# eladb3/SViT

Measured on AMD Instinct MI355X. Metric: clips/sec (fwd+bwd) SViT 16x224^2 bf16, higher is better.
Workload: dtype bf16; 1 GPU; SViT 16x224^2, 8 clips/GPU, 4 object tokens/frame, fwd+CE+bwd+clip+AdamW; global_batch=8, parallelism=dp1, ranks_seen=1, forced_dp=False, launch=hip-graph replay, input=fp32 clips, resident in the replayed step's input buffers, hip_library=svit_amd/lib/libsvit_hip.so

## Files before the change

include/svit_hip.h:

```cpp
#ifndef SVIT_HIP_H
#define SVIT_HIP_H
#include <stdint.h>
#ifdef __cplusplus
extern "C" {
#endif

#define SVIT_HEAD_DIM 96

int svit_version(void);
const char* svit_arch(void);

enum {
  SVIT_EPI_BF16 = 0,
  SVIT_EPI_GELU = 1,
  SVIT_EPI_RESID = 2,
  SVIT_EPI_F32 = 3,
  SVIT_EPI_DGELU = 4,
  SVIT_EPI_RELQ = 5
};
typedef struct {
  const void* A; int32_t lda;
  const void* W; int32_t ldw;
  const float* bias;
  void* out; int32_t ldo;
  void* out2; int32_t ldo2;
  const void* aux; int32_t ldaux;
  const float* row_scale; int32_t rows_per_sample;
  int32_t M, N, K;
  int32_t epilogue; int32_t accumulate;
  int32_t remap_L, remap_N, remap_off;
  const int32_t* relq_map;
  void* relq_out; int32_t relq_ld;
  int32_t relq_extra, relq_rows;
  float relq_scale;
} svit_gemm_args;
int svit_gemm_nt(const svit_gemm_args* args, void* stream);
int svit_gemm_tn(const void* A, int lda, const void* B, int ldb, float* dW, int lddw,
                 int M, int N, int K, int splits, float* dbias ,
                 void* stream);
#define SVIT_TN_GROUP_MAX 16
typedef struct {
  const void* A; const void* B; float* dW; float* dbias;
  int32_t lda, ldb, lddw, M, N, K;
} svit_tn_problem;
int svit_gemm_tn_grouped(const svit_tn_problem* probs, int count, void* stream);
int svit_gemm_tn_grouped_ex(const svit_tn_problem* probs, int count, int ordered, void* stream);
int svit_gemm_tn_grouped_slab(const svit_tn_problem* probs, int count, float* workspace,
                              int64_t workspace_floats, void* stream);
int64_t svit_gemm_tn_grouped_workspace(const svit_tn_problem* probs, int count);
int svit_colsum_bf16(const void* A, int lda, float* out, int M, int N, void* stream);

int svit_cast_f32_bf16(const float* src, void* dst, int64_t n, void* stream);
int svit_table_interp(const float* M, int rows, int J, const float* tables, float* out32, void* out16, void* stream);
typedef struct svit_table_interp_job {
  const float* M;
  const float* tables;
  float* out32;
  void* out16;
  int32_t rows, J;
} svit_table_interp_job;
int svit_table_interp_batched(const svit_table_interp_job* jobs_dev, int n_jobs, int max_rows, void* stream);
int svit_transpose_cast_batched(const float* src_base, void* dst_base, const int64_t* table,
                                int n_mats, int max_tiles, void* stream);
int svit_transpose_bf16_batched(const void* src_base, void* dst_base, const int64_t* table,
                                int n_mats, int max_tiles, void* stream);
int svit_pad_cast_rows(const float* src, void* dst, int R, int C, int ldd, void* stream);
int svit_scale_cast(const float* src, void* dst, const float* row_scale, int rows_per_sample,
                    int64_t rows, int cols, int gather_L, int gather_N, int gather_off,
                    void* stream);

int svit_reduce_defer(int on, void* stream);
int svit_reduce_flush(void* stream);
int svit_reduce_reset(void* stream);

int svit_layernorm_fwd(const float* x, const float* gamma, const float* beta, void* y_bf16,
                       float* y_f32, float* mean, float* rstd, int64_t rows, int C, float eps,
                       void* stream);
int svit_layernorm_bwd(const void* dy , int dy_is_bf16,
                       const float* x, const float* gamma, const float* mean,
                       const float* rstd, const float* dres, float* dx, void* dx_bf16,
                       const float* row_scale, int rows_per_sample, float* dgamma,
                       float* dbeta, int64_t rows, int C, float* workspace,
                       int64_t workspace_floats, void* stream);

int svit_im2col_patch(const float* video, void* cols, int B, int T, int H, int W, void* stream);
int svit_im2col_patch_u8(const uint8_t* frames, int64_t frames_bytes, const void* lut,
                         const int32_t* crops, void* cols, int B, int T, int Hs, int Ws, int S,
                         void* stream);
int svit_mixup_clips(float* x, const void* mix, int B, int planes, int H, int W, void* stream);
int svit_im2col_patch_u8_mix(const uint8_t* frames, int64_t frames_bytes, const float* lut_f32,
                             const int32_t* crops, const void* mix, void* cols, int B, int T, int Hs,
                             int Ws, int S, void* stream);
int svit_fill_special_tokens(float* x, const float* cls, const float* objq, const float* pos_t,
                             int B, int N, int L, int Tx, int O, int C, int add_pos, void* stream);
int svit_special_token_grads(const float* dx, float* g_cls, float* g_obj, float* g_pos, int B, int N,
                             int L, int Tx, int O, int C, int add_pos, void* stream);

typedef struct {
  const void* qkv; int32_t which;
  const float* conv_w;
  const float* gamma; const float* beta;
  void* out; int32_t ld_out;
  void* pre; float* mean; float* rstd;
  int32_t B, heads, T, H, W, n_obj;
  int32_t stride_hw;
  int32_t mode;
  float eps;
  float out_scale;
  const void* relq_R; const int32_t* relq_map; int32_t relq_lpad; float relq_scale;
} svit_pool_args;
int svit_pool_ln_fwd(const svit_pool_args* a, void* stream);

typedef struct {
  const void* d_main; int32_t main_is_f32; int32_t ld_main;
  const void* d_res; const void* d_extra;
  const void* pre; const float* mean; const float* rstd; const float* gamma;
  void* dpre; float* dgamma; float* dbeta;
  int32_t B, heads, Nout;
  float* workspace; int64_t workspace_floats;
  int32_t main_parts; int64_t main_part_stride;
  int32_t extra_is_bf16;
} svit_pool_ln_bwd_args;
int svit_pool_ln_bwd(const svit_pool_ln_bwd_args* a, void* stream);
typedef struct {
  const void* dpre; const float* conv_w; void* dqkv; int32_t which;
  int32_t B, heads, T, H, W, n_obj, stride_hw;
} svit_pool_dgrad_args;
typedef struct {
  const void* dpre; const void* qkv; int32_t which; float* dw;
  int32_t B, heads, T, H, W, n_obj, stride_hw;
  float* workspace; int64_t workspace_floats;
} svit_pool_wgrad_args;
int svit_pool_ln_fwd_qkv(const svit_pool_args* args3, void* stream);
int svit_pool_weight_sel(const float* src_base, const int64_t* src_off, uint32_t* dst, int n_tables,
                         void* stream);
int svit_pool_ln_fwd_qkv_sel(const svit_pool_args* args3, const uint32_t* const* sel3, void* stream);
int svit_pool_ln_bwd_qkv(const svit_pool_ln_bwd_args* args3, void* stream);
#ifdef SVIT_DIAG_POOL_STREAMING
int svit_pool_conv_dgrad(const svit_pool_dgrad_args* a, void* stream);
int svit_pool_conv_wgrad(const svit_pool_wgrad_args* a, void* stream);
int svit_pool_conv_dgrad_qkv(const svit_pool_dgrad_args* args3, void* stream);
int svit_pool_conv_wgrad_qkv(const svit_pool_wgrad_args* args3, void* stream);
#endif
int svit_pool_conv_bwd_qkv(const svit_pool_dgrad_args* dgrad3, const svit_pool_wgrad_args* wgrad3,
                           void* stream);
int64_t svit_pool_conv_bwd_workspace(const svit_pool_dgrad_args* dgrad3);

typedef struct {
  void* qa; int32_t ld;
  const float* rel_h; const float* rel_w; const float* rel_t;
  const int32_t* idx_h; const int32_t* idx_w; const int32_t* idx_t;
  int32_t B, heads, qt, qh, qw, kt, kh, kw, n_obj;
  float inv_scale;
} svit_relq_args;
int svit_relpos_q_fwd(const svit_relq_args* a, void* stream);
typedef struct {
  const void* qa; const void* dqa; int32_t ld;
  const float* rel_h; const float* rel_w; const float* rel_t;
  const int32_t* idx_h; const int32_t* idx_w; const int32_t* idx_t;
  float* dq_extra;
  float* drel_h; float* drel_w; float* drel_t;
  int32_t rows_h, rows_w, rows_t;
  int32_t B, heads, qt, qh, qw, kt, kh, kw, n_obj;
  float inv_scale;
  float* workspace; int64_t workspace_floats;
} svit_relq_bwd_args;
int svit_relpos_q_bwd(const svit_relq_bwd_args* a, void* stream);
typedef struct {
  const void* P; int32_t ldp; void* qa; int32_t ld;
  const int32_t* idx_h; const int32_t* idx_w; const int32_t* idx_t;
  int32_t row_h, row_w, row_t;
  int32_t B, heads, qt, qh, qw, kt, kh, kw, n_obj;
  float inv_scale;
} svit_relq_gather_args;
int svit_relpos_gather(const svit_relq_gather_args* a, void* stream);
typedef struct {
  const void* dqa; int32_t ld; void* D; int32_t ldd;
  const int32_t* idx_h; const int32_t* idx_w; const int32_t* idx_t;
  int32_t off_h, off_w, off_t;
  int32_t B, heads, qt, qh, qw, kt, kh, kw, n_obj;
  float inv_scale;
} svit_relq_scatter_args;
int svit_relpos_scatter(const svit_relq_scatter_args* a, void* stream);

typedef struct {
  const void* qa; const void* ka; const void* v; void* ctx; float* lse2;
  int32_t B, heads, Nq, Nk, DA; float scale; int32_t bias_cols;
} svit_attn_fwd_args;
int svit_attn_fwd(const svit_attn_fwd_args* a, void* stream);
typedef struct {
  const void* qa; const void* ka; const void* v; const void* ctx; const void* dctx;
  const float* lse2; float* delta;
  void* dqa;
  float* dk; float* dv;
  int32_t B, heads, Nq, Nk, DA, q_splits; float scale;
  int32_t bias_cols;
  void* relD; int32_t relD_ld; const int32_t* relD_map; float relD_scale;
  const void* relR; float* relX;
} svit_attn_bwd_args;
int svit_attn_bwd(const svit_attn_bwd_args* a, void* stream);
int svit_attn_bwd_parts(const svit_attn_bwd_args* a);

int svit_maxpool_fwd(const float* x, float* y, uint8_t* idx, int B, int T, int H, int W,
                     int n_obj, int C, void* stream);
int svit_maxpool_bwd(const float* dy, const uint8_t* idx, float* dx, int B, int T, int H, int W,
                     int n_obj, int C, void* stream);
int svit_maxpool_bwd_bf16(const float* dy, const uint8_t* idx, void* dx_bf16, int B, int T, int H, int W,
                          int n_obj, int C, void* stream);

int svit_sumsq(const float* g, int64_t n, float* sumsq, float* workspace,
               int64_t workspace_floats, void* stream);
int svit_adamw_step(float* p, const float* g, float* m, float* v, int64_t n, const float* sumsq,
                    float max_norm, float lr, float beta1, float beta2, float eps, float wd,
                    int step, float grad_scale, void* stream);

typedef struct {
  float lr[2], weight_decay[2];
  float max_norm, clip_value, grad_scale, reserved;
} svit_step_host;
typedef struct {
  int64_t applied, skipped;
  int32_t consecutive, apply;
  float coef, bc1, bc2_sqrt, sumsq, grad_norm, reserved;
} svit_step_dev;

int svit_adamw_bias_table(float beta1, float beta2, float* table, int64_t capacity, int64_t* n_entries);

int svit_step_guard(const float* g, int64_t n, const svit_step_host* host_rec, svit_step_dev* dev_rec,
                    const float* bias_table, int64_t table_entries, float* workspace, int64_t workspace_floats,
                    void* stream);
int svit_adamw_step_guarded(float* p, const float* g, float* m, float* v, int64_t n, int64_t n_decay,
                            const svit_step_host* host_rec, const svit_step_dev* dev_rec, float beta1, float beta2,
                            float eps, void* stream);

typedef struct {
  const float* tokens; int32_t B, N, C, T, O;
  const float* keep;
  const float* w_proj; const float* b_proj; int32_t n_cls;
  const float* w_box; const float* b_box;
  const float* w_bce; const float* b_bce;
  const float* w_con; const float* b_con;
  float* logits; float* boxes; float* contact; float* xobj;
} svit_head_args;
int svit_head_fwd(const svit_head_args* a, void* stream);
typedef struct {
  svit_head_args f;
  const float* dlogits; const float* dboxes; const float* dcontact; const float* dxobj;
  float* dtokens;
  float* gw_proj; float* gb_proj; float* gw_box; float* gb_box; float* gw_bce; float* gb_bce; float* gw_con; float* gb_con;
  int32_t ordered;
} svit_head_bwd_args;
int svit_head_bwd(const svit_head_bwd_args* g, void* stream);

int svit_haog_loss(const float* pred, const float* tar, const float* contact,
                   const int64_t* contact_tar, float* losses, float* g_l1, float* g_bce,
                   float* g_giou, float* g_contact, int R, int Rc, void* stream);
int svit_haog_loss_bwd(const float* upstream, const float* g_l1, const float* g_bce,
                       const float* g_giou, const float* g_contact, float* dpred,
                       float* dcontact, int R, int Rc, void* stream);

int svit_ce_loss(const float* logits, const int64_t* labels, int B, int C, float* loss, float* dlogits, void* stream);
int svit_ce_loss_soft(const float* logits, const float* target, const int64_t* labels, const void* mix, float on,
                      float off, int B, int C, float* loss, float* dlogits, void* stream);
int svit_step_draws(uint64_t* state, const float* keep, int n_blocks, int per_block, float* scales,
                    int n_drop, float p_drop, float* drop, void* stream);

int svit_ensemble_update(const float* preds, const int64_t* labels, const int64_t* clip_ids,
                         int N, int C, int num_clips, int num_videos, int mode, int repeat,
                         float* video_preds, int64_t* video_labels, int64_t* clip_count,
                         int* err, void* stream);
int svit_topk_correct(const float* video_preds, const int64_t* video_labels, int V, int C,
                      const int* ks, int nk, int* counts, int* err, void* stream);
int svit_debug_set(int key, int val);
int svit_debug_set_tn(int step_us_x100, int atomic_tbs_x100);
int svit_debug_set_tn_tile(int mode);
int svit_debug_set_pool(int key, int val);
int svit_debug_pool_bwd_path(void);
int svit_attn_debug_set(int key, int val);
int svit_debug_reset(void);
#ifdef __cplusplus
}
#endif
#endif
```

svit_amd/csrc/gemm_epilogue.h:

```cpp
#pragma once
#include "common.h"
#ifndef SVIT_EPI_AHEAD
#define SVIT_EPI_AHEAD 1
#endif
#include "../../include/svit_hip.h"

template <bool WAVE_PRIVATE>
__device__ __forceinline__ void nt_epi_sync() {
  if constexpr (WAVE_PRIVATE) asm volatile("s_waitcnt lgkmcnt(0)" ::: "memory");
  else __syncthreads();
}

template <int RB, int NB, int EPI, bool WAVE_PRIVATE = false>
__device__ __forceinline__ void nt_epilogue_wide(const svit_gemm_args& p, f32x16_t (&acc)[RB][NB],
                                                 unsigned char* smem, int m0, int n0, int wm, int wn,
                                                 int lane, int wave) {
  constexpr int WN = 32 * NB, EP_LD = WN + 4, GPR = 4 * NB;
  float* stg = (float*)smem + wave * (16 * EP_LD);
  uint4 aux_ring[3][NB];
  auto fetch_aux = [&](int ih, uint4 (&dst)[NB]) {
    const int i = ih >> 1, half = ih & 1;
#pragma unroll
    for (int it = 0; it < NB; ++it) {
      const int idx = lane + 64 * it, rl = idx / GPR, c8 = idx % GPR;
      const int row = m0 + wm * 32 * RB + i * 32 + half * 16 + rl, col = n0 + wn * WN + c8 * 8;
      dst[it] = make_uint4(0, 0, 0, 0);
      if (row < p.M && col < p.N) dst[it] = *(const uint4*)((const bf16_t*)p.aux + (size_t)row * p.ldaux + col);
    }
  };
  float4 bias_r[NB][2];
#pragma unroll
  for (int it = 0; it < NB; ++it) {
    const int col = n0 + wn * WN + ((lane + 64 * it) % GPR) * 8;
    bias_r[it][0] = bias_r[it][1] = make_float4(0.f, 0.f, 0.f, 0.f);
    if (p.bias && col < p.N) {
      bias_r[it][0] = *(const float4*)(p.bias + col);
      bias_r[it][1] = *(const float4*)(p.bias + col + 4);
    }
  }
  constexpr int AHEAD = SVIT_EPI_AHEAD;
  if (EPI == SVIT_EPI_DGELU) {
    fetch_aux(0, aux_ring[0]);
    if (AHEAD > 1 && 2 * RB > 1) fetch_aux(1, aux_ring[1]);
  }
#pragma unroll
  for (int ih = 0; ih < 2 * RB; ++ih) {
    const int i = ih >> 1, half = ih & 1;
#pragma unroll
    for (int j = 0; j < NB; ++j)
#pragma unroll
      for (int rr = 0; rr < 8; ++rr)
        stg[((rr & 3) + 8 * (rr >> 2) + 4 * (lane >> 5)) * EP_LD + j * 32 + (lane & 31)] =
            acc[i][j][half * 8 + rr];
    if (EPI == SVIT_EPI_DGELU && ih + AHEAD < 2 * RB) fetch_aux(ih + AHEAD, aux_ring[(ih + AHEAD) % 3]);
    nt_epi_sync<WAVE_PRIVATE>();
#pragma unroll
    for (int it = 0; it < NB; ++it) {
      const int idx = lane + 64 * it, rl = idx / GPR, c8 = idx % GPR;
      const int row = m0 + wm * 32 * RB + i * 32 + half * 16 + rl, col = n0 + wn * WN + c8 * 8;
      if (row >= p.M || col >= p.N) continue;
      const float4 v0 = *(const float4*)(stg + rl * EP_LD + c8 * 8), v1 = *(const float4*)(stg + rl * EP_LD + c8 * 8 + 4);
      const float4 b0 = bias_r[it][0], b1 = bias_r[it][1];
      float v[8] = {v0.x + b0.x, v0.y + b0.y, v0.z + b0.z, v0.w + b0.w, v1.x + b1.x, v1.y + b1.y, v1.z + b1.z, v1.w + b1.w};
      uint4 o;
      if constexpr (EPI == SVIT_EPI_BF16) {
        o.x = pack_bf16x2(v[0], v[1]); o.y = pack_bf16x2(v[2], v[3]);
        o.z = pack_bf16x2(v[4], v[5]); o.w = pack_bf16x2(v[6], v[7]);
      } else if constexpr (EPI == SVIT_EPI_GELU) {
        float a[8], d[8];
#pragma unroll
        for (int e = 0; e < 8; ++e) gelu_fwd_grad(v[e], &a[e], &d[e]);
        if (p.out2) {
          uint4 o2;
          o2.x = pack_bf16x2(d[0], d[1]); o2.y = pack_bf16x2(d[2], d[3]);
          o2.z = pack_bf16x2(d[4], d[5]); o2.w = pack_bf16x2(d[6], d[7]);
          *(uint4*)((bf16_t*)p.out2 + (size_t)row * p.ldo2 + col) = o2;
        }
        o.x = pack_bf16x2(a[0], a[1]); o.y = pack_bf16x2(a[2], a[3]);
        o.z = pack_bf16x2(a[4], a[5]); o.w = pack_bf16x2(a[6], a[7]);
      } else {
        const uint4 h = aux_ring[ih % 3][it];
        o.x = pack_bf16x2(v[0] * lo_bf16(h.x), v[1] * hi_bf16(h.x));
        o.y = pack_bf16x2(v[2] * lo_bf16(h.y), v[3] * hi_bf16(h.y));
        o.z = pack_bf16x2(v[4] * lo_bf16(h.z), v[5] * hi_bf16(h.z));
        o.w = pack_bf16x2(v[6] * lo_bf16(h.w), v[7] * hi_bf16(h.w));
      }
      *(uint4*)((bf16_t*)p.out + (size_t)row * p.ldo + col) = o;
    }
    if (ih + 1 < 2 * RB) nt_epi_sync<WAVE_PRIVATE>();
  }
}

template <int RB, int NB>
__device__ __forceinline__ void nt_epilogue_relq(const svit_gemm_args& p, f32x16_t (&acc)[RB][NB],
                                                 unsigned char* smem, int m0, int n0, int wm, int wn,
                                                 int lane, int wave) {
  constexpr int WN = 32 * NB, EP_LD = WN + 4;
  constexpr int MAXV = 16;
  float* stg = (float*)smem + wave * (16 * EP_LD);
  const int extra = p.relq_extra, sh = extra == 64 ? 6 : 5;
  const int nv = 16 * extra / 64;
  const int c_lo = n0 + wn * WN;
  bf16_t* qa = (bf16_t*)p.relq_out;
  int cols[2 * RB][MAXV];
#pragma unroll
  for (int ih = 0; ih < 2 * RB; ++ih) {
    const int row0 = m0 + wm * 32 * RB + (ih >> 1) * 32 + (ih & 1) * 16;
    const int tok0 = row0 % p.relq_rows;
#pragma unroll
    for (int it = 0; it < MAXV; ++it) {
      const int e = it * 64 + lane, rl = e >> sh, j = e & (extra - 1);
      cols[ih][it] = -2;
      if (it < nv && row0 + rl < p.M) {
        int tok = tok0 + rl;
        while (tok >= p.relq_rows) tok -= p.relq_rows;
        cols[ih][it] = p.relq_map[tok * extra + j];
      }
    }
  }
#pragma unroll
  for (int ih = 0; ih < 2 * RB; ++ih) {
    const int i = ih >> 1, half = ih & 1;
#pragma unroll
    for (int j = 0; j < NB; ++j)
#pragma unroll
      for (int rr = 0; rr < 8; ++rr)
        stg[((rr & 3) + 8 * (rr >> 2) + 4 * (lane >> 5)) * EP_LD + j * 32 + (lane & 31)] =
            acc[i][j][half * 8 + rr];
    nt_epi_sync<true>();
    const int row0 = m0 + wm * 32 * RB + i * 32 + half * 16;
#pragma unroll
    for (int it = 0; it < MAXV; ++it) {
      const int e = it * 64 + lane, rl = e >> sh, j = e & (extra - 1), col = cols[ih][it];
      if (col == -2) continue;
      const size_t o = (size_t)(row0 + rl) * p.relq_ld + 96 + j;
      if (col < 0) {
        if (c_lo == 0) qa[o] = 0;
      } else if (col >= c_lo && col < c_lo + WN) {
        qa[o] = f32_to_bf16(bf16_to_f32(f32_to_bf16(stg[rl * EP_LD + col - c_lo])) * p.relq_scale);
      }
    }
    if (ih + 1 < 2 * RB) nt_epi_sync<true>();
  }
}

template <int RB, int NB, int EPI, bool WAVE_PRIVATE = false>
__device__ __forceinline__ void nt_epilogue(const svit_gemm_args& p, f32x16_t (&acc)[RB][NB],
                                            unsigned char* smem, int m0, int n0, int wm, int wn,
                                            int lane, int wave) {
  if constexpr (EPI == SVIT_EPI_RELQ) {
    nt_epilogue_relq<RB, NB>(p, acc, smem, m0, n0, wm, wn, lane, wave);
    return;
  }
  if constexpr (EPI == SVIT_EPI_BF16 || EPI == SVIT_EPI_GELU || EPI == SVIT_EPI_DGELU) {
    const bool rows16 = (p.ldo % 8 == 0) && (EPI != SVIT_EPI_GELU || !p.out2 || p.ldo2 % 8 == 0) &&
                        (EPI != SVIT_EPI_DGELU || p.ldaux % 8 == 0);
    if (rows16) {
      nt_epilogue_wide<RB, NB, EPI, WAVE_PRIVATE>(p, acc, smem, m0, n0, wm, wn, lane, wave);
      return;
    }
  }
  constexpr int WN = 32 * NB;
  constexpr int EP_LD = WN + 4;
  constexpr int NIT = 2 * NB;
  constexpr bool HAS_AUX = (EPI == SVIT_EPI_RESID || EPI == SVIT_EPI_DGELU || EPI == SVIT_EPI_F32);
  float* stg = (float*)smem + wave * (16 * EP_LD);
  float4 aux_ring[3][NIT];
  constexpr int AHEAD = SVIT_EPI_AHEAD;
  const bool use_aux = HAS_AUX && (EPI != SVIT_EPI_F32 || p.accumulate);
  auto out_row = [&](int row) -> size_t {
    if (EPI == SVIT_EPI_F32 && p.remap_L > 0)
      return (size_t)(row / p.remap_L) * p.remap_N + p.remap_off + (row % p.remap_L);
    return (size_t)row;
  };
  auto fetch_aux = [&](int ih, float4 (&dst)[NIT]) {
    const int i = ih >> 1, half = ih & 1;
#pragma unroll
    for (int it = 0; it < NIT; ++it) {
      const int idx = lane + 64 * it;
      const int rl = idx / (8 * NB), c4 = idx % (8 * NB);
      const int row = m0 + wm * 32 * RB + i * 32 + half * 16 + rl;
      const int col = n0 + wn * WN + c4 * 4;
      dst[it] = make_float4(0.f, 0.f, 0.f, 0.f);
      if (row >= p.M || col >= p.N) continue;
      if constexpr (EPI == SVIT_EPI_RESID) {
        dst[it] = *(const float4*)((const float*)p.aux + (size_t)row * p.ldaux + col);
      } else if constexpr (EPI == SVIT_EPI_DGELU) {
        const uint2 h = *(const uint2*)((const bf16_t*)p.aux + (size_t)row * p.ldaux + col);
        dst[it].x = __uint_as_float(h.x);
        dst[it].y = __uint_as_float(h.y);
      } else if constexpr (EPI == SVIT_EPI_F32) {
        dst[it] = *(const float4*)((const float*)p.out + out_row(row) * p.ldo + col);
      }
    }
  };
  float4 bias_r[NIT];
#pragma unroll
  for (int it = 0; it < NIT; ++it) {
    const int col = n0 + wn * WN + ((lane + 64 * it) % (8 * NB)) * 4;
    bias_r[it] = make_float4(0.f, 0.f, 0.f, 0.f);
    if (p.bias && col < p.N) bias_r[it] = *(const float4*)(p.bias + col);
  }
  float rs_lo = 1.f, rs_hi = 1.f;
  int rs_boundary = 0x7fffffff;
  const bool rs_fast = EPI == SVIT_EPI_RESID && p.row_scale && p.rows_per_sample >= 32 * RB;
  if (rs_fast) {
    const int r_first = min(m0 + wm * 32 * RB, p.M - 1), r_last = min(r_first + 32 * RB - 1, p.M - 1);
    rs_lo = p.row_scale[r_first / p.rows_per_sample];
    rs_hi = p.row_scale[r_last / p.rows_per_sample];
    rs_boundary = (r_first / p.rows_per_sample + 1) * p.rows_per_sample;
  }
  if (use_aux) {
    fetch_aux(0, aux_ring[0]);
    if (AHEAD > 1 && 2 * RB > 1) fetch_aux(1, aux_ring[1]);
  }
#pragma unroll
  for (int ih = 0; ih < 2 * RB; ++ih) {
    const int i = ih >> 1, half = ih & 1;
#pragma unroll
    for (int j = 0; j < NB; ++j)
#pragma unroll
      for (int rr = 0; rr < 8; ++rr)
        stg[((rr & 3) + 8 * (rr >> 2) + 4 * (lane >> 5)) * EP_LD + j * 32 + (lane & 31)] =
            acc[i][j][half * 8 + rr];
    if (use_aux && ih + AHEAD < 2 * RB) fetch_aux(ih + AHEAD, aux_ring[(ih + AHEAD) % 3]);
    nt_epi_sync<WAVE_PRIVATE>();
#pragma unroll
    for (int it = 0; it < NIT; ++it) {
      const int idx = lane + 64 * it;
      const int rl = idx / (8 * NB), c4 = idx % (8 * NB);
      const int row = m0 + wm * 32 * RB + i * 32 + half * 16 + rl;
      const int col = n0 + wn * WN + c4 * 4;
      if (row >= p.M || col >= p.N) continue;
      float4 v = *(const float4*)(stg + rl * EP_LD + c4 * 4);
      {
        const float4 b = bias_r[it];
        v.x += b.x; v.y += b.y; v.z += b.z; v.w += b.w;
      }
      if constexpr (EPI == SVIT_EPI_BF16) {
        uint2 o;
        o.x = pack_bf16x2(v.x, v.y); o.y = pack_bf16x2(v.z, v.w);
        *(uint2*)((bf16_t*)p.out + (size_t)row * p.ldo + col) = o;
      } else if constexpr (EPI == SVIT_EPI_GELU) {
        float a0, a1, a2, a3, d0, d1, d2, d3;
        gelu_fwd_grad(v.x, &a0, &d0); gelu_fwd_grad(v.y, &a1, &d1);
        gelu_fwd_grad(v.z, &a2, &d2); gelu_fwd_grad(v.w, &a3, &d3);
        uint2 o;
        if (p.out2) {
          o.x = pack_bf16x2(d0, d1); o.y = pack_bf16x2(d2, d3);
          *(uint2*)((bf16_t*)p.out2 + (size_t)row * p.ldo2 + col) = o;
        }
        o.x = pack_bf16x2(a0, a1); o.y = pack_bf16x2(a2, a3);
        *(uint2*)((bf16_t*)p.out + (size_t)row * p.ldo + col) = o;
      } else if constexpr (EPI == SVIT_EPI_RESID) {
        const float s = rs_fast ? (row < rs_boundary ? rs_lo : rs_hi)
                                : (p.row_scale ? p.row_scale[row / p.rows_per_sample] : 1.f);
        const float4 res = aux_ring[ih % 3][it];
        float4 o;
        o.x = res.x + s * v.x; o.y = res.y + s * v.y; o.z = res.z + s * v.z; o.w = res.w + s * v.w;
        *(float4*)((float*)p.out + (size_t)row * p.ldo + col) = o;
      } else if constexpr (EPI == SVIT_EPI_F32) {
        float4* o = (float4*)((float*)p.out + out_row(row) * p.ldo + col);
        if (p.accumulate) {
          const float4 old = aux_ring[ih % 3][it];
          v.x += old.x; v.y += old.y; v.z += old.z; v.w += old.w;
        }
        *o = v;
      } else if constexpr (EPI == SVIT_EPI_DGELU) {
        const uint32_t hx = __float_as_uint(aux_ring[ih % 3][it].x), hy = __float_as_uint(aux_ring[ih % 3][it].y);
        uint2 o;
        o.x = pack_bf16x2(v.x * lo_bf16(hx), v.y * hi_bf16(hx));
        o.y = pack_bf16x2(v.z * lo_bf16(hy), v.w * hi_bf16(hy));
        *(uint2*)((bf16_t*)p.out + (size_t)row * p.ldo + col) = o;
      }
    }
    if (ih + 1 < 2 * RB) nt_epi_sync<WAVE_PRIVATE>();
  }
}
```

svit_amd/csrc/gemm_nt.hip:

```cpp
#include "gemm_epilogue.h"
#include "attn_common.h"

namespace {

template <int BK>
__device__ __forceinline__ int nt_lds_off(int r, int ch) {
  if constexpr (BK == 32) return r * 64 + 16 * (ch ^ ((r >> 2) & 3));
  else return (r >> 4) * 2048 + (r & 7) * 256 + ((r >> 3) & 1) * 128 + 16 * (ch ^ (r & 7));
}

template <int N>
__device__ __forceinline__ void wait_vmcnt() {
  asm volatile("s_waitcnt vmcnt(%0)" ::"n"(N) : "memory");
}

template <int RB, int NB, int WAVES_M, int WAVES_N, int STAGES, int EPI, int BK2>
__global__ __launch_bounds__(WAVES_M* WAVES_N * 64, (WAVES_M * WAVES_N > 4 ? 1 : 2)) void
gemm_nt_v2_kernel(svit_gemm_args p) {
  constexpr int NT = WAVES_M * WAVES_N * 64;
  constexpr int BM = 32 * RB * WAVES_M, WN = 32 * NB, BN = WN * WAVES_N;
  constexpr int CPR = BK2 / 8;
  constexpr int RPR = NT / CPR;
  constexpr int ROWS = (BM + BN + RPR - 1) / RPR * RPR;
  constexpr int STAGE_BYTES = ROWS * BK2 * 2;
  constexpr int PER = ROWS * CPR / NT;
  extern __shared__ __attribute__((aligned(16))) unsigned char smem[];

  const int tid = threadIdx.x, lane = tid & 63, wave = tid >> 6;
  const int wm = wave / WAVES_N, wn = wave % WAVES_N;
  const int nwg = gridDim.x * gridDim.y, lin = blockIdx.y * gridDim.x + blockIdx.x;
  const int xq = nwg >> 3, xr = nwg & 7, xcd = lin & 7;
  const int wgid = (xcd < xr ? xcd * (xq + 1) : xr * (xq + 1) + (xcd - xr) * xq) + (lin >> 3);
  const int m0 = (wgid / gridDim.x) * BM, n0 = (wgid % gridDim.x) * BN;

  const bf16_t* src[PER];
#pragma unroll
  for (int i = 0; i < PER; ++i) {
    const int q = tid + i * NT;
    int row, ch;
    if constexpr (BK2 == 32) {
      row = q >> 2;
      ch = (q & 3) ^ ((row >> 2) & 3);
    } else {
      const int line = q >> 4;
      row = (line >> 3) * 16 + ((q >> 3) & 1) * 8 + (line & 7);
      ch = (q & 7) ^ (row & 7);
    }
    if (row < BM) {
      const int gr = min(m0 + row, p.M - 1);
      src[i] = (const bf16_t*)p.A + (size_t)gr * p.lda + ch * 8;
    } else {
      const int gr = min(n0 + row - BM, p.N - 1);
      src[i] = (const bf16_t*)p.W + (size_t)gr * p.ldw + ch * 8;
    }
  }
  auto issue = [&](int kt, int stage) {
    unsigned char* base = smem + stage * STAGE_BYTES + wave * 1024;
#pragma unroll
    for (int i = 0; i < PER; ++i)
      __builtin_amdgcn_global_load_lds(
          (const __attribute__((address_space(1))) void*)(src[i] + kt * BK2),
          (__attribute__((address_space(3))) void*)(base + i * (NT * 16)), 16, 0, 0);
  };

  f32x16_t acc[RB][NB];
#pragma unroll
  for (int i = 0; i < RB; ++i)
#pragma unroll
    for (int j = 0; j < NB; ++j)
#pragma unroll
      for (int r = 0; r < 16; ++r) acc[i][j][r] = 0.f;

  const int nk = p.K / BK2;
#pragma unroll
  for (int s = 0; s < STAGES - 1; ++s)
    if (s < nk) issue(s, s);

  const int a_row = wm * 32 * RB + (lane & 31);
  const int w_row = BM + wn * WN + (lane & 31);
  for (int kt = 0; kt < nk; ++kt) {
    if (kt + STAGES - 2 < nk) wait_vmcnt<(STAGES - 2) * PER>();
    else wait_vmcnt<0>();
    __builtin_amdgcn_s_barrier();
    if (kt + STAGES - 1 < nk) issue(kt + STAGES - 1, (kt + STAGES - 1) % STAGES);
    const unsigned char* st = smem + (kt % STAGES) * STAGE_BYTES;
    bf16x8_t af[BK2 / 16][RB], wf[BK2 / 16][NB];
#pragma unroll
    for (int ks = 0; ks < BK2 / 16; ++ks) {
      const int ch = 2 * ks + (lane >> 5);
#pragma unroll
      for (int i = 0; i < RB; ++i) {
        const int r = a_row + i * 32;
        af[ks][i] = *(const bf16x8_t*)(st + nt_lds_off<BK2>(r, ch));
      }
#pragma unroll
      for (int j = 0; j < NB; ++j) {
        const int r = w_row + j * 32;
        wf[ks][j] = *(const bf16x8_t*)(st + nt_lds_off<BK2>(r, ch));
      }
    }
    __builtin_amdgcn_sched_barrier(0);
#pragma unroll
    for (int ks = 0; ks < BK2 / 16; ++ks)
#pragma unroll
      for (int i = 0; i < RB; ++i)
#pragma unroll
        for (int j = 0; j < NB; ++j) acc[i][j] = mfma32(af[ks][i], wf[ks][j], acc[i][j]);
    __builtin_amdgcn_sched_barrier(0);
  }
  __syncthreads();
  nt_epilogue<RB, NB, EPI, true>(p, acc, smem, m0, n0, wm, wn, lane, wave);
}

template <int RB, int NB, int WAVES_M, int WAVES_N, int STAGES, int BK2 = 32>
int launch_v2(const svit_gemm_args& a, hipStream_t st) {
  constexpr int BM = 32 * RB * WAVES_M, BN = 32 * NB * WAVES_N;
  constexpr int NT = WAVES_M * WAVES_N * 64;
  constexpr int RPR = NT / (BK2 / 8);
  size_t lds = (size_t)STAGES * ((BM + BN + RPR - 1) / RPR * RPR) * BK2 * 2;
  const size_t lds_epi = (size_t)WAVES_M * WAVES_N * 16 * (32 * NB + 4) * sizeof(float);
  if (lds < lds_epi) lds = lds_epi;
  dim3 grid((a.N + BN - 1) / BN, (a.M + BM - 1) / BM);
  static SvitOnce once[6];
#define SVIT_V2_ATTR(E)                                                                              \
  if (int rc = svit_max_lds_once(once[E], (const void*)gemm_nt_v2_kernel<RB, NB, WAVES_M, WAVES_N, STAGES, E, BK2>, lds)) \
    return rc
  SVIT_V2_ATTR(SVIT_EPI_BF16); SVIT_V2_ATTR(SVIT_EPI_GELU); SVIT_V2_ATTR(SVIT_EPI_RESID);
  SVIT_V2_ATTR(SVIT_EPI_F32); SVIT_V2_ATTR(SVIT_EPI_DGELU); SVIT_V2_ATTR(SVIT_EPI_RELQ);
#undef SVIT_V2_ATTR
#define SVIT_V2_CASE(E)                                                                       \
  case E:                                                                                     \
    hipLaunchKernelGGL((gemm_nt_v2_kernel<RB, NB, WAVES_M, WAVES_N, STAGES, E, BK2>), grid, dim3(NT), \
                       lds, st, a);                                                           \
    break;
  switch (a.epilogue) {
    SVIT_V2_CASE(SVIT_EPI_BF16)
    SVIT_V2_CASE(SVIT_EPI_GELU)
    SVIT_V2_CASE(SVIT_EPI_RESID)
    SVIT_V2_CASE(SVIT_EPI_F32)
    SVIT_V2_CASE(SVIT_EPI_DGELU)
    SVIT_V2_CASE(SVIT_EPI_RELQ)
    default:
      return SVIT_ERR_ARG;
  }
#undef SVIT_V2_CASE
  SVIT_LAUNCH_CHECK();
  return SVIT_OK;
}

template <int NL, int BM, int BN, int STAGES>
__device__ __forceinline__ void nt_ring_loader(const svit_gemm_args& p, unsigned char* smem, int lw, int lane,
                                               int m0, int n0, int nk) {
  constexpr int PIECES = (BM + BN) / 8;
  constexpr int PER = (PIECES + NL - 1) / NL;
  constexpr int STAGE_BYTES = (BM + BN) * 128;
  const bf16_t* src[PER];
  auto piece_of = [&](int i) { return min(lw + NL * i, PIECES - 1); };
#pragma unroll
  for (int i = 0; i < PER; ++i) {
    const int q = piece_of(i) * 64 + lane, line = q >> 4;
    const int row = (line >> 3) * 16 + ((q >> 3) & 1) * 8 + (line & 7);
    const int ch = (q & 7) ^ (row & 7);
    if (row < BM) src[i] = (const bf16_t*)p.A + (size_t)min(m0 + row, p.M - 1) * p.lda + ch * 8;
    else src[i] = (const bf16_t*)p.W + (size_t)min(n0 + row - BM, p.N - 1) * p.ldw + ch * 8;
  }
  auto issue = [&](int kt) {
    unsigned char* st = smem + (kt % STAGES) * STAGE_BYTES;
#pragma unroll
    for (int i = 0; i < PER; ++i)
      __builtin_amdgcn_global_load_lds((const __attribute__((address_space(1))) void*)(src[i] + kt * 64),
                                       (__attribute__((address_space(3))) void*)(st + piece_of(i) * 1024), 16, 0, 0);
  };
#pragma unroll
  for (int s = 0; s < STAGES; ++s)
    if (s < nk) issue(s);
  for (int kt = 0; kt < nk; ++kt) {
    const int younger = (kt == 0 ? min(STAGES - 1, nk - 1) : min(kt + STAGES - 2, nk - 1) - kt);
    attn::static_for<0, STAGES>([&](auto Y) {
      if (younger == decltype(Y)::value) wait_vmcnt<decltype(Y)::value * PER>();
    });
    __builtin_amdgcn_s_barrier();
    if (kt >= 1 && kt - 1 + STAGES < nk) issue(kt - 1 + STAGES);
  }
}

template <int RB, int NB, int WAVES_M, int WAVES_N, int NL, int STAGES, int EPI>
__global__ __launch_bounds__((WAVES_M * WAVES_N + NL) * 64, 1) void gemm_nt_ring_kernel(svit_gemm_args p) {
  using attn::Int;
  constexpr int NC = WAVES_M * WAVES_N;
  constexpr int BM = 32 * RB * WAVES_M, WN = 32 * NB, BN = WN * WAVES_N;
  static_assert(BM % 16 == 0 && BN % 16 == 0, "a 1-KiB piece must not straddle A and W rows");
  constexpr int STAGE_BYTES = (BM + BN) * 128;
  extern __shared__ __attribute__((aligned(16))) unsigned char smem[];

  const int lane = threadIdx.x & 63;
  const int wave = __builtin_amdgcn_readfirstlane(threadIdx.x >> 6);
  const int nwg = gridDim.x * gridDim.y, lin = blockIdx.y * gridDim.x + blockIdx.x;
  const int xq = nwg >> 3, xr = nwg & 7, xcd = lin & 7;
  const int wgid = (xcd < xr ? xcd * (xq + 1) : xr * (xq + 1) + (xcd - xr) * xq) + (lin >> 3);
  const int m0 = (wgid / gridDim.x) * BM, n0 = (wgid % gridDim.x) * BN;
  const int nk = p.K / 64;

  if (wave >= NC) {
    nt_ring_loader<NL, BM, BN, STAGES>(p, smem, wave - NC, lane, m0, n0, nk);
    return;
  }

  const int wm = wave / WAVES_N, wn = wave % WAVES_N;
  f32x16_t acc[RB][NB];
#pragma unroll
  for (int i = 0; i < RB; ++i)
#pragma unroll
    for (int j = 0; j < NB; ++j)
#pragma unroll
      for (int r = 0; r < 16; ++r) acc[i][j][r] = 0.f;

  const int l31 = lane & 31, x7 = lane & 7;
  unsigned fa[4], fw[4];
#pragma unroll
  for (int ks = 0; ks < 4; ++ks) {
    const unsigned lp = (unsigned)((l31 >> 4) * 2048 + x7 * 256 + ((l31 >> 3) & 1) * 128 +
                                   32 * (ks ^ (x7 >> 1)) + 16 * ((lane >> 5) ^ (x7 & 1)));
    fa[ks] = (unsigned)(size_t)smem + lp + (unsigned)(wm * 2 * RB) * 2048u;
    fw[ks] = (unsigned)(size_t)smem + lp + (unsigned)((BM + wn * WN) / 16) * 2048u;
  }
  bf16x8_t fr[2][RB + NB];
  auto reads = [&](auto KS, auto BUF, unsigned so, auto HALF) {
    constexpr int ks = decltype(KS)::value, b = decltype(BUF)::value, h = decltype(HALF)::value;
    attn::static_for<0, RB + NB>([&](auto F) {
      constexpr int f = decltype(F)::value;
      if constexpr ((f / 2) == h) {
        if constexpr (f < RB) attn::lds_read128<f * 4096>(fr[b][f], fa[ks] + so);
        else attn::lds_read128<(f - RB) * 4096>(fr[b][f], fw[ks] + so);
      }
    });
  };
  constexpr int NH = (RB + NB + 1) / 2;
  auto release = [&](auto BUF) {
    constexpr int b = decltype(BUF)::value;
    attn::static_for<0, RB + NB>([&](auto F) { attn::lgkm_release1<0>(fr[b][decltype(F)::value]); });
  };
  auto substep = [&](auto BUF, auto NEXT_KS, unsigned next_so, bool do_reads) {
    constexpr int b = decltype(BUF)::value;
    attn::static_for<0, RB * NB>([&](auto Q) {
      constexpr int q = decltype(Q)::value, i = q / NB, j = q % NB;
      acc[i][j] = mfma32(fr[b][i], fr[b][RB + j], acc[i][j]);
      if constexpr (q < NH) {
        if (do_reads) reads(NEXT_KS, Int<1 - b>{}, next_so, Int<q>{});
      }
      __builtin_amdgcn_sched_barrier(0);
    });
  };

  __builtin_amdgcn_s_barrier();
  attn::static_for<0, NH>([&](auto H) { reads(Int<0>{}, Int<0>{}, 0u, H); });
  release(Int<0>{});
  for (int kt = 0; kt < nk; ++kt) {
    const unsigned so = (unsigned)((kt % STAGES) * STAGE_BYTES);
    const unsigned so_next = (unsigned)(((kt + 1) % STAGES) * STAGE_BYTES);
    const bool more = kt + 1 < nk;
    substep(Int<0>{}, Int<1>{}, so, true);
    release(Int<1>{});
    substep(Int<1>{}, Int<2>{}, so, true);
    release(Int<0>{});
    substep(Int<0>{}, Int<3>{}, so, true);
    release(Int<1>{});
    if (more) __builtin_amdgcn_s_barrier();
    substep(Int<1>{}, Int<0>{}, so_next, more);
    if (more) release(Int<0>{});
  }
  unsigned char* epi = smem + (nk >= 2 ? (nk - 2) % STAGES : 1) * STAGE_BYTES;
  nt_epilogue<RB, NB, EPI, true>(p, acc, epi, m0, n0, wm, wn, lane, wave);
}

template <int RB, int NB, int WAVES_M, int WAVES_N, int NL, int STAGES>
int launch_ring(const svit_gemm_args& a, hipStream_t st) {
  constexpr int BM = 32 * RB * WAVES_M, BN = 32 * NB * WAVES_N, NT = (WAVES_M * WAVES_N + NL) * 64;
  constexpr size_t lds = (size_t)STAGES * (BM + BN) * 128;
  static_assert((size_t)WAVES_M * WAVES_N * 16 * (32 * NB + 4) * sizeof(float) <= (size_t)(BM + BN) * 128, "epilogue staging fits a slot");
  static_assert(lds <= 160 * 1024, "LDS");
  dim3 grid((a.N + BN - 1) / BN, (a.M + BM - 1) / BM);
  static SvitOnce once[5];
#define SVIT_RING_ATTR(E)                                                                              \
  if (int rc = svit_max_lds_once(once[E], (const void*)gemm_nt_ring_kernel<RB, NB, WAVES_M, WAVES_N, NL, STAGES, E>, lds)) \
    return rc
  SVIT_RING_ATTR(SVIT_EPI_BF16); SVIT_RING_ATTR(SVIT_EPI_GELU); SVIT_RING_ATTR(SVIT_EPI_RESID);
  SVIT_RING_ATTR(SVIT_EPI_F32); SVIT_RING_ATTR(SVIT_EPI_DGELU);
#undef SVIT_RING_ATTR
#define SVIT_RING_CASE(E)                                                                       \
  case E:                                                                                       \
    hipLaunchKernelGGL((gemm_nt_ring_kernel<RB, NB, WAVES_M, WAVES_N, NL, STAGES, E>), grid, dim3(NT), lds, st, a); \
    break;
  switch (a.epilogue) {
    SVIT_RING_CASE(SVIT_EPI_BF16)
    SVIT_RING_CASE(SVIT_EPI_GELU)
    SVIT_RING_CASE(SVIT_EPI_RESID)
    SVIT_RING_CASE(SVIT_EPI_F32)
    SVIT_RING_CASE(SVIT_EPI_DGELU)
    default:
      return SVIT_ERR_ARG;
  }
#undef SVIT_RING_CASE
  SVIT_LAUNCH_CHECK();
  return SVIT_OK;
}
}

static void ring_choice(const svit_gemm_args& a, int* cfg, int* stages) {
  const long tm = (a.M + 127) / 128;
  const long t192 = a.N % 192 == 0 ? tm * (a.N / 192) : 0, t96 = tm * ((a.N + 95) / 96);
  constexpr int k_min5 = 1024, t_max6 = 256, s6 = 4;
  if (t96 <= t_max6 && a.K >= 768) { *cfg = 6, *stages = (t96 > 256 ? 2 : s6); return; }
  if (t192 >= 160 && a.N <= 768 && a.K >= k_min5) { *cfg = 5, *stages = 3; return; }
}

extern "C" int svit_gemm_nt(const svit_gemm_args* args, void* stream) {
  if (!args || !args->A || !args->W) return SVIT_ERR_ARG;
  const svit_gemm_args& a = *args;
  const bool relq = a.epilogue == SVIT_EPI_RELQ;
  if (!relq && !a.out) return SVIT_ERR_ARG;
  if (relq) {
    if (!a.relq_map || !a.relq_out || (a.relq_extra != 32 && a.relq_extra != 64) || a.relq_rows < 1 ||
        a.relq_ld < 96 + a.relq_extra || a.bias)
      return SVIT_ERR_ARG;
  }
  if (a.M <= 0 || a.N <= 0 || a.K <= 0 || a.K % 32 != 0 || a.N % 96 != 0) return SVIT_ERR_SHAPE;
  if (a.lda % 8 != 0 || a.ldw % 8 != 0 || a.lda < a.K || a.ldw < a.K || (!relq && a.ldo < a.N))
    return SVIT_ERR_ALIGN;
  if (((uintptr_t)a.A | (uintptr_t)a.W) & 15) return SVIT_ERR_ALIGN;
  if (!relq && (a.ldo % 4 != 0 || ((uintptr_t)a.out & 15))) return SVIT_ERR_ALIGN;
  if (a.bias && ((uintptr_t)a.bias & 15)) return SVIT_ERR_ALIGN;
  if (a.aux && (a.ldaux % 4 != 0 || ((uintptr_t)a.aux & 15))) return SVIT_ERR_ALIGN;
  if (a.out2 && (a.ldo2 % 4 != 0 || ((uintptr_t)a.out2 & 15))) return SVIT_ERR_ALIGN;
  if ((a.epilogue == SVIT_EPI_RESID || a.epilogue == SVIT_EPI_DGELU) && !a.aux) return SVIT_ERR_ARG;
  if (a.epilogue == SVIT_EPI_RESID && a.row_scale && a.rows_per_sample <= 0) return SVIT_ERR_ARG;
  hipStream_t st = (hipStream_t)stream;
  const int force_raw = svit_knob(SVIT_K_NT_CFG), force_stages = svit_knob(SVIT_K_NT_STAGES);
  const bool no_ring = force_raw == 8 || svit_knob(SVIT_K_NT_BK) != 0;
  const int force_cfg = force_raw == 8 ? -1 : force_raw;
  if (a.K % 64 == 0 && !relq && ((force_cfg < 0 && !no_ring) || (force_cfg >= 5 && force_cfg <= 7))) {
    int cfg = force_cfg, rs = force_stages;
    if (cfg < 0) ring_choice(a, &cfg, &rs);
    if (cfg >= 5) {
      if (!rs) rs = 3;
#define SVIT_RING_PICK(RB, NB, WM, WN)                                         \
  do {                                                                         \
    if (rs == 2) return launch_ring<RB, NB, WM, WN, 4, 2>(a, st);              \
    if (rs == 3) return launch_ring<RB, NB, WM, WN, 4, 3>(a, st);              \
    return launch_ring<RB, NB, WM, WN, 4, 4>(a, st);                           \
  } while (0)
      if (cfg == 5) SVIT_RING_PICK(2, 3, 2, 2);
      if (cfg == 6) SVIT_RING_PICK(1, 3, 4, 1);
      SVIT_RING_PICK(2, 2, 2, 2);
#undef SVIT_RING_PICK
    }
  }
  bool big = a.N % 192 == 0 && (long)((a.M + 127) / 128) * (a.N / 192) >= 256;
  if (force_cfg == 0 && a.N % 192 == 0) big = true;
  if (force_cfg == 2) big = false;
  const int stages = force_stages ? force_stages : (a.K >= 2048 ? 4 : 2);
  bool sq = a.N % 128 == 0 && a.N >= 1024 && a.K <= 512 &&
            (long)((a.M + 127) / 128) * (a.N / 128) <= 2048;
  if (force_cfg == 4) sq = a.N % 128 == 0;
  else if (force_cfg >= 0) sq = false;
  const int force_bk = svit_knob(SVIT_K_NT_BK);
  bool bk64 = a.K % 64 == 0 && a.N <= 768 && a.K >= 384;
  if (force_bk) bk64 = force_bk == 64 && a.K % 64 == 0;
  if (bk64 && force_cfg < 0 && !force_stages) return launch_v2<1, 3, 4, 1, 2, 64>(a, st);
#define SVIT_NT_PICK(RB, NB, WM, WN)                                           \
  do {                                                                         \
    if (bk64) {                                                                \
      if (stages == 2) return launch_v2<RB, NB, WM, WN, 2, 64>(a, st);         \
      if (stages == 3) return launch_v2<RB, NB, WM, WN, 3, 64>(a, st);         \
      return launch_v2<RB, NB, WM, WN, 4, 64>(a, st);                          \
    }                                                                          \
    if (stages == 2) return launch_v2<RB, NB, WM, WN, 2, 32>(a, st);           \
    if (stages == 3) return launch_v2<RB, NB, WM, WN, 3, 32>(a, st);           \
    return launch_v2<RB, NB, WM, WN, 4, 32>(a, st);                            \
  } while (0)
  {
    constexpr int one_round = 1;
    const long t160 = a.N % 256 == 0 ? (long)((a.M + 159) / 160) * (a.N / 256) : 0;
    const long t192 = a.N % 192 == 0 ? (long)((a.M + 191) / 192) * (a.N / 192) : 0;
    const long t128 = (long)((a.M + 127) / 128) * ((a.N + 191) / 192);
    const bool auto_ok = force_cfg < 0 && one_round && !force_stages && !force_bk && a.K <= 512 && t128 > 512;
    if (force_cfg == 9 || (auto_ok && t160 > 256 && t160 <= 512)) {
      if (a.N % 256 == 0) return launch_v2<5, 2, 1, 4, 2, 32>(a, st);
    }
    if (force_cfg == 10 || (auto_ok && t192 > 256 && t192 <= 512)) {
      if (a.N % 192 == 0) return launch_v2<3, 3, 2, 2, 2, 32>(a, st);
    }
  }
  if (sq) SVIT_NT_PICK(2, 2, 2, 2);
  if (big) SVIT_NT_PICK(2, 3, 2, 2);
  SVIT_NT_PICK(1, 3, 4, 1);
#undef SVIT_NT_PICK
}
```

svit_amd/csrc/norm.hip:

```cpp
#include <algorithm>
#include <cstdlib>
#include "common.h"
#include "../../include/svit_hip.h"

namespace {
constexpr int LN_MAX_CHUNKS = 3;

template <bool HALF>
__device__ __forceinline__ float row_sum(float v) {
#pragma unroll
  for (int o = HALF ? 16 : 32; o > 0; o >>= 1) v += __shfl_xor(v, o, 64);
  return v;
}

template <int NCH, bool HALF>
__global__ __launch_bounds__(256) void ln_fwd_kernel(const float* __restrict__ x,
                                                     const float* __restrict__ gamma,
                                                     const float* __restrict__ beta,
                                                     bf16_t* __restrict__ y16,
                                                     float* __restrict__ y32,
                                                     float* __restrict__ mean_out,
                                                     float* __restrict__ rstd_out, int64_t rows,
                                                     int C, float eps) {
  constexpr int LW = HALF ? 32 : 64;
  constexpr int RPW = HALF ? 2 : 1;
  const int lane = threadIdx.x & 63, wave = threadIdx.x >> 6;
  const int lr = lane & (LW - 1), sub = HALF ? (lane >> 5) : 0;
  const int nch = C >> 2;
  const float inv_c = 1.0f / (float)C;
  float4 g[NCH], bt[NCH];
#pragma unroll
  for (int i = 0; i < NCH; ++i) {
    const int c = lr + i * LW;
    g[i] = bt[i] = make_float4(0.f, 0.f, 0.f, 0.f);
    if (c < nch) { g[i] = ((const float4*)gamma)[c]; bt[i] = ((const float4*)beta)[c]; }
  }
  const int64_t stride = (int64_t)gridDim.x * 4 * RPW;
  for (int64_t row0 = ((int64_t)blockIdx.x * 4 + wave) * RPW + sub; row0 < rows; row0 += 2 * stride) {
    float4 v[2][NCH];
    int64_t rk[2];
    bool has[2];
#pragma unroll
    for (int k = 0; k < 2; ++k) {
      has[k] = row0 + k * stride < rows;
      rk[k] = has[k] ? row0 + k * stride : row0;
#pragma unroll
      for (int i = 0; i < NCH; ++i) {
        const int c = lr + i * LW;
        v[k][i] = make_float4(0.f, 0.f, 0.f, 0.f);
        if (c < nch) v[k][i] = ((const float4*)(x + rk[k] * C))[c];
      }
    }
#pragma unroll
    for (int k = 0; k < 2; ++k) {
      float s = 0.f;
#pragma unroll
      for (int i = 0; i < NCH; ++i) s += v[k][i].x + v[k][i].y + v[k][i].z + v[k][i].w;
      const float mean = row_sum<HALF>(s) * inv_c;
      float sq = 0.f;
#pragma unroll
      for (int i = 0; i < NCH; ++i) {
        if (lr + i * LW < nch) {
          const float a = v[k][i].x - mean, b = v[k][i].y - mean, cc = v[k][i].z - mean,
                      d = v[k][i].w - mean;
          sq += a * a + b * b + cc * cc + d * d;
        }
      }
      const float rstd = rsqrtf(row_sum<HALF>(sq) * inv_c + eps);
      if (!has[k]) continue;
      if (lr == 0) {
        if (mean_out) mean_out[rk[k]] = mean;
        if (rstd_out) rstd_out[rk[k]] = rstd;
      }
#pragma unroll
      for (int i = 0; i < NCH; ++i) {
        const int c = lr + i * LW;
        if (c < nch) {
          float4 o;
          o.x = (v[k][i].x - mean) * rstd * g[i].x + bt[i].x;
          o.y = (v[k][i].y - mean) * rstd * g[i].y + bt[i].y;
          o.z = (v[k][i].z - mean) * rstd * g[i].z + bt[i].z;
          o.w = (v[k][i].w - mean) * rstd * g[i].w + bt[i].w;
          if (y16) {
            uint2 pk;
            pk.x = pack_bf16x2(o.x, o.y);
            pk.y = pack_bf16x2(o.z, o.w);
            *(uint2*)(y16 + rk[k] * C + c * 4) = pk;
          }
          if (y32) ((float4*)(y32 + rk[k] * C))[c] = o;
        }
      }
    }
  }
}

template <int NCH, bool HALF, bool DYB>
__global__ __launch_bounds__(256) void ln_bwd_kernel(const void* __restrict__ dy_,
                                                     const float* __restrict__ x,
                                                     const float* __restrict__ gamma,
                                                     const float* __restrict__ mean_in,
                                                     const float* __restrict__ rstd_in,
                                                     const float* __restrict__ dres,
                                                     float* __restrict__ dx,
                                                     bf16_t* __restrict__ dx16,
                                                     const float* __restrict__ row_scale,
                                                     int rows_per_sample,
                                                     float* __restrict__ partial,
                                                     int64_t rows, int C) {
  constexpr int LW = HALF ? 32 : 64;
  constexpr int RPW = HALF ? 2 : 1;
  __shared__ float red[4][2][NCH * 256];
  const int lane = threadIdx.x & 63, wave = threadIdx.x >> 6;
  const int lr = lane & (LW - 1), sub = HALF ? (lane >> 5) : 0;
  const int nch = C >> 2;
  const float inv_c = 1.0f / (float)C;
  float4 gacc[NCH], bacc[NCH], gm[NCH];
#pragma unroll
  for (int i = 0; i < NCH; ++i) {
    gacc[i] = make_float4(0.f, 0.f, 0.f, 0.f);
    bacc[i] = make_float4(0.f, 0.f, 0.f, 0.f);
    const int c = lr + i * LW;
    gm[i] = (c < nch) ? ((const float4*)gamma)[c] : make_float4(0.f, 0.f, 0.f, 0.f);
  }
  const int64_t stride = (int64_t)gridDim.x * 4 * RPW;
  for (int64_t row0 = ((int64_t)blockIdx.x * 4 + wave) * RPW + sub; row0 < rows; row0 += 2 * stride) {
    float4 xv[2][NCH], dv[2][NCH], rv[2][NCH];
    float mean[2], rstd[2], sc16[2];
    int64_t rowk[2];
    bool has[2];
#pragma unroll
    for (int k = 0; k < 2; ++k) {
      has[k] = row0 + k * stride < rows;
      rowk[k] = has[k] ? row0 + k * stride : row0;
      mean[k] = mean_in[rowk[k]];
      rstd[k] = rstd_in[rowk[k]];
      sc16[k] = (dx16 && row_scale) ? row_scale[rowk[k] / rows_per_sample] : 1.f;
#pragma unroll
      for (int i = 0; i < NCH; ++i) {
        const int c = lr + i * LW;
        xv[k][i] = dv[k][i] = rv[k][i] = make_float4(0.f, 0.f, 0.f, 0.f);
        if (c < nch) {
          xv[k][i] = ((const float4*)(x + rowk[k] * C))[c];
          if (DYB) {
            const uint2 h = ((const uint2*)((const bf16_t*)dy_ + rowk[k] * C))[c];
            dv[k][i] = make_float4(lo_bf16(h.x), hi_bf16(h.x), lo_bf16(h.y), hi_bf16(h.y));
          } else {
            dv[k][i] = ((const float4*)((const float*)dy_ + rowk[k] * C))[c];
          }
          if (dres) rv[k][i] = ((const float4*)(dres + rowk[k] * C))[c];
        }
      }
    }
#pragma unroll
    for (int k = 0; k < 2; ++k) {
      float4 xh[NCH], g[NCH];
      float s1 = 0.f, s2 = 0.f;
      const float live = has[k] ? 1.f : 0.f;
#pragma unroll
      for (int i = 0; i < NCH; ++i) {
        const float4 d = dv[k][i];
        xh[i].x = (xv[k][i].x - mean[k]) * rstd[k]; xh[i].y = (xv[k][i].y - mean[k]) * rstd[k];
        xh[i].z = (xv[k][i].z - mean[k]) * rstd[k]; xh[i].w = (xv[k][i].w - mean[k]) * rstd[k];
        if (lr + i * LW >= nch) xh[i] = make_float4(0.f, 0.f, 0.f, 0.f);
        gacc[i].x += live * d.x * xh[i].x; gacc[i].y += live * d.y * xh[i].y;
        gacc[i].z += live * d.z * xh[i].z; gacc[i].w += live * d.w * xh[i].w;
        bacc[i].x += live * d.x; bacc[i].y += live * d.y;
        bacc[i].z += live * d.z; bacc[i].w += live * d.w;
        g[i].x = d.x * gm[i].x; g[i].y = d.y * gm[i].y;
        g[i].z = d.z * gm[i].z; g[i].w = d.w * gm[i].w;
        s1 += g[i].x + g[i].y + g[i].z + g[i].w;
        s2 += g[i].x * xh[i].x + g[i].y * xh[i].y + g[i].z * xh[i].z + g[i].w * xh[i].w;
      }
      s1 = row_sum<HALF>(s1) * inv_c;
      s2 = row_sum<HALF>(s2) * inv_c;
      if (!has[k]) continue;
#pragma unroll
      for (int i = 0; i < NCH; ++i) {
        const int c = lr + i * LW;
        if (c < nch) {
          float4 o;
          o.x = rstd[k] * (g[i].x - s1 - xh[i].x * s2) + rv[k][i].x;
          o.y = rstd[k] * (g[i].y - s1 - xh[i].y * s2) + rv[k][i].y;
          o.z = rstd[k] * (g[i].z - s1 - xh[i].z * s2) + rv[k][i].z;
          o.w = rstd[k] * (g[i].w - s1 - xh[i].w * s2) + rv[k][i].w;
          ((float4*)(dx + rowk[k] * C))[c] = o;
          if (dx16) {
            uint2 h;
            h.x = pack_bf16x2(o.x * sc16[k], o.y * sc16[k]);
            h.y = pack_bf16x2(o.z * sc16[k], o.w * sc16[k]);
            ((uint2*)(dx16 + rowk[k] * C))[c] = h;
          }
        }
      }
    }
  }
  if (HALF) {
#pragma unroll
    for (int i = 0; i < NCH; ++i) {
      gacc[i].x += __shfl_xor(gacc[i].x, 32, 64); gacc[i].y += __shfl_xor(gacc[i].y, 32, 64);
      gacc[i].z += __shfl_xor(gacc[i].z, 32, 64); gacc[i].w += __shfl_xor(gacc[i].w, 32, 64);
      bacc[i].x += __shfl_xor(bacc[i].x, 32, 64); bacc[i].y += __shfl_xor(bacc[i].y, 32, 64);
      bacc[i].z += __shfl_xor(bacc[i].z, 32, 64); bacc[i].w += __shfl_xor(bacc[i].w, 32, 64);
    }
  }
#pragma unroll
  for (int i = 0; i < NCH; ++i) {
    const int c = lr + i * LW;
    if (c < nch && sub == 0) {
      *(float4*)&red[wave][0][c * 4] = gacc[i];
      *(float4*)&red[wave][1][c * 4] = bacc[i];
    }
  }
  __syncthreads();
  float* prow = partial + (size_t)blockIdx.x * 2 * C;
  for (int c = threadIdx.x; c < C; c += 256) {
    prow[c] = red[0][0][c] + red[1][0][c] + red[2][0][c] + red[3][0][c];
    prow[C + c] = red[0][1][c] + red[1][1][c] + red[2][1][c] + red[3][1][c];
  }
}
}

extern "C" int svit_layernorm_fwd(const float* x, const float* gamma, const float* beta,
                                  void* y_bf16, float* y_f32, float* mean, float* rstd,
                                  int64_t rows, int C, float eps, void* stream) {
  if (!x || !gamma || !beta || (!y_bf16 && !y_f32)) return SVIT_ERR_ARG;
  if (rows <= 0 || C <= 0 || C % 4 != 0 || C > 768) return SVIT_ERR_SHAPE;
  constexpr int rpb_f = 8;
  int64_t blocks = (rows + rpb_f - 1) / rpb_f;
  if (blocks > 16384) blocks = 16384;
  if (blocks < 1) blocks = 1;
#define SVIT_LN_FWD(NCH, HALF)                                                                \
  hipLaunchKernelGGL((ln_fwd_kernel<NCH, HALF>), dim3((unsigned)blocks), dim3(256), 0,           \
                     (hipStream_t)stream, x, gamma, beta, (bf16_t*)y_bf16, y_f32, mean, rstd,    \
                     rows, C, eps)
  if (C <= 128) SVIT_LN_FWD(1, true);
  else if (C <= 256) SVIT_LN_FWD(1, false);
  else if (C <= 512) SVIT_LN_FWD(2, false);
  else SVIT_LN_FWD(3, false);
#undef SVIT_LN_FWD
  SVIT_LAUNCH_CHECK();
  return SVIT_OK;
}

extern "C" int svit_layernorm_bwd(const void* dy, int dy_is_bf16, const float* x, const float* gamma,
                                  const float* mean, const float* rstd, const float* dres,
                                  float* dx, void* dx_bf16, const float* row_scale,
                                  int rows_per_sample, float* dgamma, float* dbeta, int64_t rows,
                                  int C, float* workspace, int64_t workspace_floats,
                                  void* stream) {
  if (!dy || !x || !gamma || !mean || !rstd || !dx || !dgamma || !dbeta || !workspace)
    return SVIT_ERR_ARG;
  if (dx_bf16 && row_scale && rows_per_sample <= 0) return SVIT_ERR_ARG;
  if (rows <= 0 || C <= 0 || C % 4 != 0 || C > 768) return SVIT_ERR_SHAPE;
  constexpr int rpb = 16;
  int64_t blocks = (rows + rpb - 1) / rpb;
  if (blocks < 256) blocks = (rows + 3) / 4 < 256 ? (rows + 3) / 4 : 256;
  if (blocks > 2048) blocks = 2048;
  if (blocks > workspace_floats / (2 * C)) blocks = workspace_floats / (2 * C);
  if (blocks < 1) return SVIT_ERR_ARG;
#define SVIT_LN_BWD(NCH, HALF)                                                                  \
  do {                                                                                            \
    if (dy_is_bf16)                                                                               \
      hipLaunchKernelGGL((ln_bwd_kernel<NCH, HALF, true>), dim3((unsigned)blocks), dim3(256), 0,  \
                         (hipStream_t)stream, dy, x, gamma, mean, rstd, dres, dx,                 \
                         (bf16_t*)dx_bf16, row_scale, rows_per_sample, workspace, rows, C);       \
    else                                                                                          \
      hipLaunchKernelGGL((ln_bwd_kernel<NCH, HALF, false>), dim3((unsigned)blocks), dim3(256), 0, \
                         (hipStream_t)stream, dy, x, gamma, mean, rstd, dres, dx,                 \
                         (bf16_t*)dx_bf16, row_scale, rows_per_sample, workspace, rows, C);       \
  } while (0)
  if (C <= 128) SVIT_LN_BWD(1, true);
  else if (C <= 256) SVIT_LN_BWD(1, false);
  else if (C <= 512) SVIT_LN_BWD(2, false);
  else SVIT_LN_BWD(3, false);
#undef SVIT_LN_BWD
  SVIT_LAUNCH_CHECK();
  SvitReduceDst dst = {{dgamma, dbeta, dbeta, dbeta, dbeta, dbeta}, {C, 2 * C, 2 * C, 2 * C, 2 * C, 2 * C}};
  svit_launch_reduce(workspace, (int)blocks, 2 * C, dst, (hipStream_t)stream);
  SVIT_LAUNCH_CHECK();
  return SVIT_OK;
}
```

svit_amd/engine.py:

```python
import math

import torch

from . import arch, hip, ops
from .input import U8Clips

HD = arch.HEAD_DIM
F32, BF16 = torch.float32, torch.bfloat16
SCALE = HD ** -0.5
LOG2E = 1.4426950408889634
K_SCALE = SCALE * LOG2E


def _align(n, a=8):
    return (n + a - 1) // a * a


class FlatParams:

    def __init__(self, shapes, decay_of, device, rank_of):
        names = list(shapes)
        depth = 1 + max([int(n.split(".")[1]) for n in names if n.startswith("blocks.")] or [0])
        ranks = {n: rank_of(n, depth) for n in names}
        order = sorted(names, key=lambda n: (not decay_of(n, shapes[n]), ranks[n]))
        self.slots, off = {}, 0
        self.n_decay = 0
        self.n_ranks = depth + 2
        self.ready_ranges = [[] for _ in range(self.n_ranks)]
        for n in order:
            numel = int(math.prod(shapes[n]))
            self.slots[n] = (off, numel, tuple(shapes[n]))
            rr = self.ready_ranges[ranks[n]]
            if rr and rr[-1][1] == off:
                rr[-1] = (rr[-1][0], off + _align(numel))
            else:
                rr.append((off, off + _align(numel)))
            off += _align(numel)
            if decay_of(n, shapes[n]):
                self.n_decay = off
        self.total = off
        self.data = torch.zeros(off, device=device, dtype=F32)
        self.grad = torch.zeros(off, device=device, dtype=F32)
        self.w16 = torch.zeros(off + 96 * 96, device=device, dtype=BF16)
        self.t_slots, toff, table = {}, 0, []
        for n in order:
            if n.startswith("blocks.") and n.endswith(".weight") and len(shapes[n]) == 2:
                r, c = shapes[n]
                self.t_slots[n] = (toff, (c, r))
                table += [self.slots[n][0], toff, r, c, r]
                toff += _align(r * c)
        self.rel_slots = {}
        for n in order:
            if n.endswith("attn.rel_pos_h"):
                pre = n[:-len("attn.rel_pos_h")]
                rows = [shapes[pre + "attn.rel_pos_" + a][0] for a in "hwt"]
                offs, lpad = rel_sections(rows)
                self.rel_slots[pre] = (toff, lpad, offs)
                for a, o, r in zip("hwt", offs, rows):
                    table += [self.slots[pre + "attn.rel_pos_" + a][0], toff + o, r, HD, lpad]
                toff += _align(HD * lpad)
        pool_names = [n for n in names if ".attn.pool_" in n and n.endswith(".weight")]
        pool_names.sort(key=lambda n: (int(n.split(".")[1]), "qkv".index(n.split(".")[3][-1])))
        self.pool_sel_index = {n: i for i, n in enumerate(pool_names)}
        self.pool_sel = torch.zeros((max(1, len(pool_names)), 27 * 96), device=device, dtype=torch.int32)
        self.pool_sel_off = torch.tensor([self.slots[n][0] for n in pool_names] or [0], dtype=torch.int64,
                                         device=device)
        self.wT16 = torch.zeros(max(toff, 8), device=device, dtype=BF16)
        self.t_table = torch.tensor(table, dtype=torch.int64, device=device)
        self.n_t = len(table) // 5

    def view(self, buf, name):
        off, numel, shape = self.slots[name]
        return buf[off:off + numel].view(shape)

    def p(self, name):
        return self.view(self.data, name)

    def g(self, name):
        return self.view(self.grad, name)

    def w(self, name):
        off, numel, shape = self.slots[name]
        return self.w16[off:off + numel].view(shape)

    def wt(self, name):
        off, shape = self.t_slots[name]
        return self.wT16[off:off + shape[0] * shape[1]].view(shape)

    def rel_cat_t(self, pre):
        off, lpad, offs = self.rel_slots[pre]
        return self.wT16[off:off + HD * lpad].view(HD, lpad), lpad, offs

    def rel_tables32(self, pre):
        names = [pre + "attn.rel_pos_" + a for a in "hwt"]
        offs = [self.slots[n][0] for n in names]
        rows = [self.slots[n][2][0] for n in names]
        assert offs[1] == offs[0] + rows[0] * HD and offs[2] == offs[1] + rows[1] * HD
        return self.data[offs[0]:offs[0] + sum(rows) * HD].view(sum(rows), HD)

    def rel_cat(self, pre):
        names = [pre + "attn.rel_pos_" + a for a in "hwt"]
        offs = [self.slots[n][0] for n in names]
        rows = [self.slots[n][2][0] for n in names]
        assert offs[1] == offs[0] + rows[0] * HD and offs[2] == offs[1] + rows[1] * HD
        total = rows[0] + rows[1] + rows[2]
        lpad = (total + 95) // 96 * 96
        return (self.w16[offs[0]:offs[0] + lpad * HD].view(lpad, HD), (0, rows[0], rows[0] + rows[1]))

    def sels(self, pre):
        return [self.pool_sel[self.pool_sel_index[pre + "attn.pool_%s.weight" % r]] for r in "qkv"]

    TILED_MIN_PLANE = 2048
    SLAB_MAX_PLANE = 196

    def refresh_low_precision(self):
        ops.cast_bf16(self.data, self.w16[:self.total])
        if self.pool_sel_index:
            ops.pool_weight_sel(self.data, self.pool_sel_off, self.pool_sel)
        if self.n_t:
            ops.transpose_bf16_batched(self.w16, self.wT16, self.t_table, self.n_t, 256)


def rel_sections(rows):
    off_w = _align(rows[0])
    off_t = off_w + _align(rows[1])
    return (0, off_w, off_t), _align(off_t + rows[2], 32)


def _rel_index(q_n, k_n):
    q_ratio = max(k_n / q_n, 1.0)
    k_ratio = max(q_n / k_n, 1.0)
    d = torch.arange(q_n)[:, None] * q_ratio - torch.arange(k_n)[None, :] * k_ratio
    d = d + (k_n - 1) * k_ratio
    return d.long().to(torch.int32)


def _resize_matrix(rows_have, rows_need):
    m = torch.zeros(rows_need, rows_have)
    scale = rows_have / rows_need
    for i in range(rows_need):
        pos = max((i + 0.5) * scale - 0.5, 0.0)
        i0 = min(int(math.floor(pos)), rows_have - 1)
        i1 = min(i0 + 1, rows_have - 1)
        lam = pos - i0
        m[i, i0] += 1.0 - lam
        m[i, i1] += lam
    return m


class Engine:
    def __init__(self, plan: arch.Plan, flat: FlatParams, red_group=4):
        self.plan, self.flat = plan, flat
        self.dev = flat.data.device
        self._rel_cache = {}
        self._interp_cache = {}
        self._interp_out = {}
        self.batch_interp = True
        self._relq_cache = {}
        self.fused_scatter = True
        self.patch_w16 = torch.zeros((plan.embed_dim, 448), device=self.dev, dtype=BF16)
        self._tn = []
        self.RED_GROUP = max(1, int(red_group))
        M1 = 1024 * 1024
        self._red_ws = torch.empty(self.RED_GROUP * 18 * M1, device=self.dev, dtype=F32)
        self._red_slot = 0
        self._wgrad_need, self._wgrad_big = {}, {}
        self._red_regions = {"ln2": (0, 4 * M1), "ln1": (4 * M1, 8 * M1), "pln": (8 * M1, 9 * M1),
                             "wgrad": (9 * M1, 18 * M1)}
        self._side = None
        self._side_keep = []
        self._side_active = False
        self.overlap_wgrad = False
        self.attn_q_splits = 0
        self.deterministic = False
        self.reproducible = False
        self._capture_fork = None
        self._capture_join = None

    def refresh_weights(self):
        self.flat.refresh_low_precision()
        ops.pad_cast_rows(self.flat.p("patch_embed.proj.weight").view(self.plan.embed_dim, 441),
                          self.patch_w16)

    def _rel(self, blk, q_thw, k_thw):
        key = (blk.index, q_thw, k_thw)
        ent = self._rel_cache.get(key)
        if ent is None:
            idx = [_rel_index(q_thw[1], k_thw[1]), _rel_index(q_thw[2], k_thw[2]),
                   _rel_index(q_thw[0], k_thw[0])]
            need = [2 * max(q_thw[i], k_thw[i]) - 1 for i in (1, 2, 0)]
            have = [blk.rel_sp_rows, blk.rel_sp_rows, blk.rel_t_rows]
            mats = [None if n == h else _resize_matrix(h, n).to(self.dev) for n, h in zip(need, have)]
            mcat = None
            if any(m is not None for m in mats):
                lp = (sum(need) + 95) // 96 * 96
                mcat = torch.zeros((lp, sum(have)), device=self.dev)
                r0 = c0 = 0
                for n, h, m in zip(need, have, mats):
                    mcat[r0:r0 + n, c0:c0 + h] = torch.eye(h, device=self.dev) if m is None else m
                    r0, c0 = r0 + n, c0 + h
            ent = ([t.contiguous().to(self.dev) for t in idx], mats, mcat, tuple(need))
            self._rel_cache[key] = ent
        return ent

    def _interp_tables(self, thw, save):
        if not self.batch_interp:
            self._interp_out = {}
            return
        key = (tuple(thw), bool(save))
        ent = self._interp_cache.get(key)
        if ent is None:
            entries, outs, cur = [], {}, tuple(thw)
            for blk in self.plan.blocks:
                sq, skv = blk.stride_q[1], blk.stride_kv[1]
                q_thw = (cur[0], arch.pooled(cur[1], sq), arch.pooled(cur[2], sq))
                k_thw = (cur[0], arch.pooled(cur[1], skv), arch.pooled(cur[2], skv))
                _, _, mcat, _ = self._rel(blk, q_thw, k_thw)
                if mcat is not None:
                    r32 = torch.empty((mcat.shape[0], HD), device=self.dev, dtype=F32) if save else None
                    r16 = torch.empty((mcat.shape[0], HD), device=self.dev, dtype=BF16)
                    entries.append((mcat, self.flat.rel_tables32("blocks.%d." % blk.index), r32, r16))
                    outs[blk.index] = (r32, r16)
                cur = q_thw
            jobs = ops.table_interp_jobs(entries, self.dev) if entries else None
            ent = (jobs, max((e[0].shape[0] for e in entries), default=0), outs, entries)
            self._interp_cache[key] = ent
        jobs, max_rows, outs, _ = ent
        if jobs is not None:
            ops.table_interp_batched(jobs, max_rows)
        self._interp_out = outs

    def _relq_map(self, blk, q_thw, k_thw, idx, rows_off, n_obj, extra):
        key = (blk.index, q_thw, k_thw, tuple(rows_off), n_obj, extra)
        m = self._relq_cache.get(key)
        if m is None:
            qt, qh, qw = q_thw
            kt, kh, kw = k_thw
            ih, iw, it = (t.cpu().view(n, k) for t, n, k in zip(idx, (qh, qw, qt), (kh, kw, kt)))
            Lq = qt * qh * qw
            body = torch.full((qt, qh, qw, extra), -1, dtype=torch.int32)
            body[..., :kh] = (rows_off[0] + ih).view(1, qh, 1, kh)
            body[..., kh:kh + kw] = (rows_off[1] + iw).view(1, 1, qw, kw)
            body[..., kh + kw:kh + kw + kt] = (rows_off[2] + it).view(qt, 1, 1, kt)
            m = torch.full((1 + Lq + n_obj, extra), -1, dtype=torch.int32)
            m[1:1 + Lq] = body.view(Lq, extra)
            m = m.contiguous().to(self.dev)
            self._relq_cache[key] = m
        return m

    def _tables(self, pre, mats):
        names = (pre + "attn.rel_pos_h", pre + "attn.rel_pos_w", pre + "attn.rel_pos_t")
        out = []
        for n, m in zip(names, mats):
            t = self.flat.p(n)
            out.append(t if m is None else (m @ t).contiguous())
        return out

    def forward(self, video, drop_scales=None, save=True):
        plan, f = self.plan, self.flat
        if isinstance(video, U8Clips):
            B, _, Tx = video.shape[:3]
            cols, (To, Ho, Wo) = ops.im2col_patch_u8(video)
        else:
            if video.dim() == 4:
                video = video.unsqueeze(2)
            video = video.contiguous().to(F32)
            B, _, Tx = video.shape[:3]
            cols, (To, Ho, Wo) = ops.im2col_patch(video)
        T = plan.num_frames // plan.patch_stride[0] if Tx > 1 else Tx
        if To != T:
            raise hip.SvitHipError("clip has %d frames but cfg.DATA.NUM_FRAMES=%d" % (Tx, plan.num_frames))
        L, n_obj, C = To * Ho * Wo, Tx * plan.objects, plan.embed_dim
        N = 1 + L + n_obj
        x = torch.empty((B, N, C), device=self.dev, dtype=F32)
        ops.gemm_nt(cols, self.patch_w16, f.p("patch_embed.proj.bias"), hip.EPI_F32,
                    out=x.view(B * N, C), remap=(L, N, 1))
        ops.fill_special_tokens(x, f.p("cls_token"), f.p("object_queries"),
                                f.p("pos_embed_temporal"), L, Tx, plan.objects, Tx > 1)
        st = {"B": B, "Tx": Tx, "n_obj": n_obj, "L0": L, "cols": cols if save else None,
              "blocks": []}
        thw = (T, Ho, Wo)
        self._interp_tables(thw, save)
        hip.mark("stem")
        for blk in plan.blocks:
            ds = drop_scales[blk.index] if drop_scales is not None else None
            x, thw, sv = self._block_fwd(blk, x, thw, n_obj, ds, save)
            st["blocks"].append(sv)
            hip.mark("fwd%d" % blk.index)
        y16, y32, mean, rstd = ops.layernorm_fwd(x, f.p("norm.weight"), f.p("norm.bias"),
                                                 want_f32=True, want_bf16=False, save_stats=save)
        st.update(x_last=x if save else None, mean=mean, rstd=rstd, thw=thw)
        self._interp_out = {}
        return y32, st

    def _block_fwd(self, blk, x, thw, n_obj, ds, save):
        f = self.flat
        pre = "blocks.%d." % blk.index
        B, N, C = x.shape
        Co, h = blk.dim_out, blk.heads
        sq, skv = blk.stride_q[1], blk.stride_kv[1]
        q_thw = (thw[0], arch.pooled(thw[1], sq), arch.pooled(thw[2], sq))
        k_thw = (thw[0], arch.pooled(thw[1], skv), arch.pooled(thw[2], skv))
        Nq = 1 + q_thw[0] * q_thw[1] * q_thw[2] + n_obj
        J = k_thw[0] + k_thw[1] + k_thw[2]
        DA = HD + 32 if J <= 32 else HD + 64
        if J > 64:
            raise hip.SvitHipError("key grid %s too large for the in-MFMA rel-pos bias" % (k_thw,))
        xn, _, mean1, rstd1 = ops.layernorm_fwd(x, f.p(pre + "norm1.weight"), f.p(pre + "norm1.bias"),
                                                save_stats=save)
        xn2d = xn.view(B * N, C)
        qkv = ops.gemm_nt(xn2d, f.w(pre + "attn.qkv.weight"), f.p(pre + "attn.qkv.bias"), hip.EPI_BF16)
        idx, mats, mcat, need = self._rel(blk, q_thw, k_thw)
        if mcat is None:
            tabs = self._tables(pre, mats)
            rcat, rows_off = f.rel_cat(pre)
        else:
            if blk.index in self._interp_out:
                r32, rcat = self._interp_out[blk.index]
            else:
                r32, rcat = ops.table_interp(mcat, f.rel_tables32(pre), want_f32=save)
            rows_off = (0, need[0], need[0] + need[1])
            tabs = None if r32 is None else [r32[rows_off[0]:rows_off[0] + need[0]], r32[rows_off[1]:rows_off[1] + need[1]],
                                             r32[rows_off[2]:rows_off[2] + need[2]]]
        pools = ops.pool_ln_fwd_qkv(
            qkv, [f.p(pre + "attn.pool_%s.weight" % r).view(HD, 27) for r in "qkv"],
            [f.p(pre + "attn.norm_%s.weight" % r) for r in "qkv"],
            [f.p(pre + "attn.norm_%s.bias" % r) for r in "qkv"],
            B, h, thw, n_obj, (sq, skv, skv), (DA, DA, HD), (0, 1, 0), save=save, out_scales=(1.0, K_SCALE, 1.0),
            sels=f.sels(pre) if (thw[1] * thw[2] >= f.TILED_MIN_PLANE or thw[1] * thw[2] <= f.SLAB_MAX_PLANE)
            else None,
            relq=(rcat.contiguous(), self._relq_map(blk, q_thw, k_thw, idx, rows_off, n_obj, DA - HD), LOG2E))
        qa, ka, v = pools[0][0], pools[1][0], pools[2][0]
        ctx, lse2 = ops.attn_fwd(qa, ka, v, SCALE, bias_cols=J)
        pool_idx = None
        if blk.has_proj:
            skip = ops.gemm_nt(xn2d, f.w(pre + "proj.weight"), f.p(pre + "proj.bias"), hip.EPI_F32)
            skip = skip.view(B, N, Co)
        else:
            skip = x
        if blk.pools_q:
            skip, pool_idx = ops.maxpool_fwd(skip, thw, n_obj)
        dpa, dpm = ds if ds is not None else (None, None)
        x1 = ops.gemm_nt(ctx.view(B * Nq, Co), f.w(pre + "attn.proj.weight"), f.p(pre + "attn.proj.bias"),
                         hip.EPI_RESID, aux=skip.view(B * Nq, Co), row_scale=dpa, rows_per_sample=Nq)
        x1 = x1.view(B, Nq, Co)
        xn2, _, mean2, rstd2 = ops.layernorm_fwd(x1, f.p(pre + "norm2.weight"), f.p(pre + "norm2.bias"),
                                                 save_stats=save)
        act, dact = ops.gemm_nt(xn2.view(B * Nq, Co), f.w(pre + "mlp.fc1.weight"),
                                f.p(pre + "mlp.fc1.bias"), hip.EPI_GELU, save=save)
        x2 = ops.gemm_nt(act, f.w(pre + "mlp.fc2.weight"), f.p(pre + "mlp.fc2.bias"), hip.EPI_RESID,
                         aux=x1.view(B * Nq, Co), row_scale=dpm, rows_per_sample=Nq).view(B, Nq, Co)
        sv = None
        if save:
            sv = dict(x=x, thw=thw, q_thw=q_thw, k_thw=k_thw, mean1=mean1, rstd1=rstd1, xn=xn2d,
                      qkv=qkv, pools=pools, tabs=tabs, idx=idx, mats=mats, ctx=ctx, lse2=lse2,
                      pool_idx=pool_idx, x1=x1, mean2=mean2, rstd2=rstd2, xn2=xn2, act=act,
                      dact=dact, dpa=dpa, dpm=dpm, Nq=Nq)
        return x2, q_thw, sv

    def backward(self, st, dy, on_ready=None, ready_ranks=None):
        def ready(rank):
            if on_ready is not None:
                if ready_ranks is None or rank in ready_ranks:
                    ops.reduce_flush()
                    self._flush_tn()
                    self._join()
                on_ready(rank)
        plan, f = self.plan, self.flat
        depth = len(plan.blocks)
        last = st["blocks"][depth - 1]
        dx, dx16 = ops.layernorm_bwd(dy.contiguous(), st["x_last"], f.p("norm.weight"), st["mean"],
                                     st["rstd"], f.g("norm.weight"), f.g("norm.bias"),
                                     want_bf16=True, row_scale=last["dpm"],
                                     rows_per_sample=st["x_last"].shape[1])
        ready(0)
        hip.mark("bwd_norm")
        for blk in reversed(plan.blocks):
            below = st["blocks"][blk.index - 1] if blk.index > 0 else None
            try:
                G = self.RED_GROUP
                dx, dx16 = self._block_bwd(blk, st["blocks"][blk.index], dx, dx16, st["n_obj"], below,
                                           red_begin=blk.index % G == G - 1 or blk.index == depth - 1,
                                           red_end=blk.index % G == 0, red_slot=blk.index % G)
            except BaseException:
                ops.reduce_reset()
                self._tn = []
                raise
            hip.mark("bwd%d" % blk.index)
            ready(1 + (depth - 1 - blk.index))
        B, Tx, L, O, C = st["B"], st["Tx"], st["L0"], plan.objects, plan.embed_dim
        ops.special_token_grads(dx, f.g("cls_token"), f.g("object_queries"),
                                f.g("pos_embed_temporal") if Tx > 1 else None, L, Tx, O, Tx > 1)
        dtok = ops.scale_cast(dx, gather=(L, 1))
        self._gemm_tn(dtok, st["cols"], f.g("patch_embed.proj.weight").view(C, 441), f.g("patch_embed.proj.bias"))
        self._flush_tn()
        self._join()
        ready(depth + 1)

    def _rws(self, key):
        a, b = self._red_regions[key]
        o = self._red_slot * 18 * 1024 * 1024
        return self._red_ws[o + a:o + b]

    def _wgrad_ws(self, B, h, thw, n_obj, strides):
        key = (B, h, tuple(thw), n_obj, tuple(strides))
        need = self._wgrad_need.get(key)
        if need is None:
            need = self._wgrad_need[key] = ops.pool_conv_bwd_workspace(B, h, thw, n_obj, strides)
        ws = self._rws("wgrad")
        if need <= ws.numel():
            return ws
        big = self._wgrad_big.get(self._red_slot)
        if big is None or big.numel() < need:
            big = self._wgrad_big[self._red_slot] = torch.empty(need, device=self.dev, dtype=F32)
        return big

    def _fork(self, fn, keep):
        if not self.overlap_wgrad:
            fn()
            return
        if self._capture_fork is not None:
            self._capture_fork(fn)
            self._side_active = True
            return
        main = torch.cuda.current_stream(self.dev)
        if self._side is None:
            self._side = torch.cuda.Stream(device=self.dev)
        self._side.wait_stream(main)
        with torch.cuda.stream(self._side):
            fn()
        self._side_keep.append(keep)
        self._side_active = True

    def _join(self):
        if self._side_active and self._capture_join is not None:
            self._capture_join()
            self._side_active = False
            return
        if self._side_active:
            torch.cuda.current_stream(self.dev).wait_stream(self._side)
            self._side_keep.clear()
            self._side_active = False

    def _flush_tn(self, force=True):
        if not force and len(self._tn) <= 8:
            return
        q, self._tn = self._tn, []
        if not q:
            return
        det = self.deterministic
        if self.reproducible and not det:
            self._fork(lambda: ops.gemm_tn_grouped_slab(q, tag="tn_slab_queue"), q)
            return
        self._fork(lambda: ops.gemm_tn_grouped(q, ordered=det), q)

    def _gemm_tn(self, a, b, dw, dbias=None):
        if self.deterministic:
            ops.gemm_tn(a, b, dw, splits=1, dbias=dbias)
        elif self.reproducible:
            ops.gemm_tn_grouped_slab([(a, b, dw, dbias)], tag="tn_slab_main")
        else:
            ops.gemm_tn(a, b, dw, splits=0, dbias=dbias)

    def _linear_bwd(self, dy16, x16, wname, bname, need_dx, out=None, accumulate=False,
                    epilogue=hip.EPI_F32, aux=None):
        f = self.flat
        self._tn.append((dy16, x16, f.g(wname), f.g(bname)))
        if not need_dx:
            return None
        return ops.gemm_nt(dy16, f.wt(wname), None, epilogue, out=out, aux=aux, accumulate=accumulate)

    def _block_bwd(self, blk, sv, dx2, dy, n_obj, below, red_begin=True, red_end=True, red_slot=0):
        f = self.flat
        pre = "blocks.%d." % blk.index
        B, Nq, Co = dx2.shape
        x = sv["x"]
        N, C, h = x.shape[1], x.shape[2], blk.heads
        M, Mq = B * N, B * Nq
        sq, skv = blk.stride_q[1], blk.stride_kv[1]
        thw, q_thw, k_thw = sv["thw"], sv["q_thw"], sv["k_thw"]
        self._red_slot = red_slot
        if red_begin:
            ops.reduce_defer(True)
        dy = dy.view(Mq, Co)
        dh = self._linear_bwd(dy, sv["act"], pre + "mlp.fc2.weight", pre + "mlp.fc2.bias", True,
                              epilogue=hip.EPI_DGELU, aux=sv["dact"])
        dxn2 = self._linear_bwd(dh, sv["xn2"].view(Mq, Co), pre + "mlp.fc1.weight",
                                pre + "mlp.fc1.bias", True, epilogue=hip.EPI_BF16)
        dx1, dy = ops.layernorm_bwd(dxn2, sv["x1"], f.p(pre + "norm2.weight"), sv["mean2"],
                                    sv["rstd2"], f.g(pre + "norm2.weight"), f.g(pre + "norm2.bias"),
                                    dres=dx2, want_bf16=True, row_scale=sv["dpa"], rows_per_sample=Nq,
                                    ws=self._rws("ln2"))
        dy = dy.view(Mq, Co)
        dctx = self._linear_bwd(dy, sv["ctx"].view(Mq, Co), pre + "attn.proj.weight",
                                pre + "attn.proj.bias", True, epilogue=hip.EPI_BF16)
        (qa, preq, mq, rq), (ka, prek, mk, rk), (v, prev, mv, rv) = sv["pools"]
        tabs, mats = sv["tabs"], sv["mats"]
        names = (pre + "attn.rel_pos_h", pre + "attn.rel_pos_w", pre + "attn.rel_pos_t")
        if all(m is None for m in mats):
            rcat_t, lpad, offs = f.rel_cat_t(pre)
        else:
            offs, lpad = rel_sections([t.shape[0] for t in tabs])
            rcat = torch.zeros((lpad, HD), device=self.dev, dtype=F32)
            for o, t in zip(offs, tabs):
                rcat[o:o + t.shape[0]] = t
            rcat_t = rcat.t().contiguous().to(BF16)
        if self.fused_scatter:
            dmap = self._relq_map(blk, q_thw, k_thw, sv["idx"], offs, n_obj, qa.shape[-1] - HD)
            dqa, dk, dv, D, dq_extra = ops.attn_bwd(
                qa, ka, v, sv["ctx"], dctx.view(B, Nq, Co), sv["lse2"], SCALE,
                q_splits=1 if self.deterministic else self.attn_q_splits, bias_cols=sum(sv["k_thw"]),
                reld=(dmap, lpad, LOG2E, rcat_t if rcat_t.is_contiguous() else None, "fold"))
        else:
            dqa, dk, dv = ops.attn_bwd(qa, ka, v, sv["ctx"], dctx.view(B, Nq, Co), sv["lse2"], SCALE,
                                       q_splits=1 if self.deterministic else self.attn_q_splits,
                                       bias_cols=sum(sv["k_thw"]))
            D = ops.relpos_scatter(dqa, sv["idx"], offs, lpad, B, h, q_thw, k_thw, n_obj, LOG2E)
            dq_extra = None
        qa2 = qa.view(B * h * Nq, qa.shape[-1])
        for n, m, t, o in zip(names, mats, tabs, offs):
            rows = t.shape[0]
            if m is None:
                self._tn.append((D[:, o:o + rows], qa2[:, :HD], f.g(n), None))
            else:
                d = torch.zeros_like(t)
                self._gemm_tn(D[:, o:o + rows], qa2[:, :HD], d)
                f.g(n).add_(m.t() @ d)
        if dq_extra is None:
            dq_extra = ops.gemm_nt(D, rcat_t, None, hip.EPI_BF16)
        elif isinstance(dq_extra, str):
            dq_extra = None
        Nk = ka.shape[2]
        dqkv = torch.empty_like(sv["qkv"])
        entries = []
        for r, pre_t, mean, rstd, nout, kw in (
                ("q", preq, mq, rq, Nq, dict(d_main=dqa, ld_main=qa.shape[-1], d_res=dctx,
                                             d_extra=dq_extra)),
                ("k", prek, mk, rk, Nk, dict(d_main=dk, ld_main=HD)),
                ("v", prev, mv, rv, Nk, dict(d_main=dv, ld_main=HD))):
            entries.append(((pre_t, mean, rstd, f.p(pre + "attn.norm_%s.weight" % r),
                             f.g(pre + "attn.norm_%s.weight" % r),
                             f.g(pre + "attn.norm_%s.bias" % r), B, h, nout), kw))
        dpres = ops.pool_ln_bwd_qkv(entries, ws=self._rws("pln"))
        strides = (sq, skv, skv)
        ops.pool_conv_bwd_qkv(dpres, [f.p(pre + "attn.pool_%s.weight" % r).view(HD, 27) for r in "qkv"],
                              dqkv, sv["qkv"],
                              [f.g(pre + "attn.pool_%s.weight" % r).view(HD, 27) for r in "qkv"],
                              B, h, thw, n_obj, strides, ws=self._wgrad_ws(B, h, thw, n_obj, strides))
        dxn = self._linear_bwd(dqkv, sv["xn"], pre + "attn.qkv.weight", pre + "attn.qkv.bias", True,
                               epilogue=hip.EPI_F32 if blk.has_proj else hip.EPI_BF16)
        dskip = dx1
        if blk.pools_q:
            dskip = ops.maxpool_bwd(dskip, sv["pool_idx"], thw, n_obj, bf16=blk.has_proj)
        if blk.has_proj:
            ds16 = dskip.view(M, Co) if blk.pools_q else ops.scale_cast(dskip.view(M, Co))
            self._linear_bwd(ds16, sv["xn"], pre + "proj.weight", pre + "proj.bias", True, out=dxn,
                             accumulate=True)
            dskip = None
        res = ops.layernorm_bwd(dxn, x, f.p(pre + "norm1.weight"), sv["mean1"], sv["rstd1"],
                                f.g(pre + "norm1.weight"), f.g(pre + "norm1.bias"), dres=dskip,
                                want_bf16=below is not None,
                                row_scale=below["dpm"] if below is not None else None,
                                rows_per_sample=N, ws=self._rws("ln1"))
        if red_end:
            ops.reduce_defer(False)
        self._flush_tn(force=False)
        if below is None:
            return res.view(B, N, C), None
        return res[0].view(B, N, C), res[1]
```

svit_amd/hip.py:

```python
import ctypes as C
import os

import torch

_HERE = os.path.dirname(os.path.abspath(__file__))
LIB_PATH = os.environ.get("SVIT_HIP_LIB") or os.path.join(_HERE, "lib", "libsvit_hip.so")
_lib = None

vp, i32, i64, f32 = C.c_void_p, C.c_int32, C.c_int64, C.c_float

EPI_BF16, EPI_GELU, EPI_RESID, EPI_F32, EPI_DGELU, EPI_RELQ = 0, 1, 2, 3, 4, 5


class TnProblem(C.Structure):
    _fields_ = [("A", vp), ("B", vp), ("dW", vp), ("dbias", vp), ("lda", i32), ("ldb", i32),
                ("lddw", i32), ("M", i32), ("N", i32), ("K", i32)]


class GemmArgs(C.Structure):
    _fields_ = [("A", vp), ("lda", i32), ("W", vp), ("ldw", i32), ("bias", vp), ("out", vp),
                ("ldo", i32), ("out2", vp), ("ldo2", i32), ("aux", vp), ("ldaux", i32),
                ("row_scale", vp), ("rows_per_sample", i32), ("M", i32), ("N", i32), ("K", i32),
                ("epilogue", i32), ("accumulate", i32), ("remap_L", i32), ("remap_N", i32),
                ("remap_off", i32), ("relq_map", vp), ("relq_out", vp), ("relq_ld", i32),
                ("relq_extra", i32), ("relq_rows", i32), ("relq_scale", f32)]


class PoolArgs(C.Structure):
    _fields_ = [("qkv", vp), ("which", i32), ("conv_w", vp), ("gamma", vp), ("beta", vp),
                ("out", vp), ("ld_out", i32), ("pre", vp), ("mean", vp), ("rstd", vp),
                ("B", i32), ("heads", i32), ("T", i32), ("H", i32), ("W", i32), ("n_obj", i32),
                ("stride_hw", i32), ("mode", i32), ("eps", f32), ("out_scale", f32),
                ("relq_R", vp), ("relq_map", vp), ("relq_lpad", i32), ("relq_scale", f32)]


class PoolLnBwdArgs(C.Structure):
    _fields_ = [("d_main", vp), ("main_is_f32", i32), ("ld_main", i32), ("d_res", vp),
                ("d_extra", vp), ("pre", vp), ("mean", vp), ("rstd", vp), ("gamma", vp),
                ("dpre", vp), ("dgamma", vp), ("dbeta", vp), ("B", i32), ("heads", i32),
                ("Nout", i32), ("workspace", vp), ("workspace_floats", i64), ("main_parts", i32),
                ("main_part_stride", i64), ("extra_is_bf16", i32)]


class PoolDgradArgs(C.Structure):
    _fields_ = [("dpre", vp), ("conv_w", vp), ("dqkv", vp), ("which", i32), ("B", i32),
                ("heads", i32), ("T", i32), ("H", i32), ("W", i32), ("n_obj", i32),
                ("stride_hw", i32)]


class PoolWgradArgs(C.Structure):
    _fields_ = [("dpre", vp), ("qkv", vp), ("which", i32), ("dw", vp), ("B", i32), ("heads", i32),
                ("T", i32), ("H", i32), ("W", i32), ("n_obj", i32), ("stride_hw", i32),
                ("workspace", vp), ("workspace_floats", i64)]


class RelqArgs(C.Structure):
    _fields_ = [("qa", vp), ("ld", i32), ("rel_h", vp), ("rel_w", vp), ("rel_t", vp),
                ("idx_h", vp), ("idx_w", vp), ("idx_t", vp), ("B", i32), ("heads", i32),
                ("qt", i32), ("qh", i32), ("qw", i32), ("kt", i32), ("kh", i32), ("kw", i32),
                ("n_obj", i32), ("inv_scale", f32)]


class RelqBwdArgs(C.Structure):
    _fields_ = [("qa", vp), ("dqa", vp), ("ld", i32), ("rel_h", vp), ("rel_w", vp), ("rel_t", vp),
                ("idx_h", vp), ("idx_w", vp), ("idx_t", vp), ("dq_extra", vp), ("drel_h", vp),
                ("drel_w", vp), ("drel_t", vp), ("rows_h", i32), ("rows_w", i32), ("rows_t", i32),
                ("B", i32), ("heads", i32), ("qt", i32), ("qh", i32), ("qw", i32), ("kt", i32),
                ("kh", i32), ("kw", i32), ("n_obj", i32), ("inv_scale", f32),
                ("workspace", vp), ("workspace_floats", i64)]


class RelqGatherArgs(C.Structure):
    _fields_ = [("P", vp), ("ldp", i32), ("qa", vp), ("ld", i32), ("idx_h", vp), ("idx_w", vp),
                ("idx_t", vp), ("row_h", i32), ("row_w", i32), ("row_t", i32), ("B", i32),
                ("heads", i32), ("qt", i32), ("qh", i32), ("qw", i32), ("kt", i32), ("kh", i32),
                ("kw", i32), ("n_obj", i32), ("inv_scale", f32)]


class RelqScatterArgs(C.Structure):
    _fields_ = [("dqa", vp), ("ld", i32), ("D", vp), ("ldd", i32), ("idx_h", vp), ("idx_w", vp),
                ("idx_t", vp), ("off_h", i32), ("off_w", i32), ("off_t", i32), ("B", i32),
                ("heads", i32), ("qt", i32), ("qh", i32), ("qw", i32), ("kt", i32), ("kh", i32),
                ("kw", i32), ("n_obj", i32), ("inv_scale", f32)]


class AttnFwdArgs(C.Structure):
    _fields_ = [("qa", vp), ("ka", vp), ("v", vp), ("ctx", vp), ("lse2", vp), ("B", i32),
                ("heads", i32), ("Nq", i32), ("Nk", i32), ("DA", i32), ("scale", f32),
                ("bias_cols", i32)]


class AttnBwdArgs(C.Structure):
    _fields_ = [("qa", vp), ("ka", vp), ("v", vp), ("ctx", vp), ("dctx", vp), ("lse2", vp),
                ("delta", vp), ("dqa", vp), ("dk", vp), ("dv", vp), ("B", i32), ("heads", i32),
                ("Nq", i32), ("Nk", i32), ("DA", i32), ("q_splits", i32), ("scale", f32),
                ("bias_cols", i32), ("relD", vp), ("relD_ld", i32), ("relD_map", vp), ("relD_scale", f32),
                ("relR", vp), ("relX", vp)]


class HeadArgs(C.Structure):
    _fields_ = [("tokens", vp), ("B", i32), ("N", i32), ("C", i32), ("T", i32), ("O", i32), ("keep", vp),
                ("w_proj", vp), ("b_proj", vp), ("n_cls", i32), ("w_box", vp), ("b_box", vp),
                ("w_bce", vp), ("b_bce", vp), ("w_con", vp), ("b_con", vp),
                ("logits", vp), ("boxes", vp), ("contact", vp), ("xobj", vp)]


class HeadBwdArgs(C.Structure):
    _fields_ = [("f", HeadArgs), ("dlogits", vp), ("dboxes", vp), ("dcontact", vp), ("dxobj", vp), ("dtokens", vp),
                ("gw_proj", vp), ("gb_proj", vp), ("gw_box", vp), ("gb_box", vp), ("gw_bce", vp), ("gb_bce", vp),
                ("gw_con", vp), ("gb_con", vp), ("ordered", i32)]


class StepHost(C.Structure):
    _fields_ = [("lr", f32 * 2), ("weight_decay", f32 * 2), ("max_norm", f32), ("clip_value", f32),
                ("grad_scale", f32), ("reserved", f32)]


class StepDev(C.Structure):
    _fields_ = [("applied", i64), ("skipped", i64), ("consecutive", i32), ("apply", i32), ("coef", f32),
                ("bc1", f32), ("bc2_sqrt", f32), ("sumsq", f32), ("grad_norm", f32), ("reserved", f32)]


_SIGS = {
    "svit_version": (i32, []),
    "svit_arch": (C.c_char_p, []),
    "svit_gemm_nt": (i32, [C.POINTER(GemmArgs), vp]),
    "svit_gemm_tn": (i32, [vp, i32, vp, i32, vp, i32, i32, i32, i32, i32, vp, vp]),
    "svit_gemm_tn_grouped": (i32, [C.POINTER(TnProblem), i32, vp]),
    "svit_gemm_tn_grouped_ex": (i32, [C.POINTER(TnProblem), i32, i32, vp]),
    "svit_gemm_tn_grouped_slab": (i32, [C.POINTER(TnProblem), i32, vp, i64, vp]),
    "svit_gemm_tn_grouped_workspace": (i64, [C.POINTER(TnProblem), i32]),
    "svit_colsum_bf16": (i32, [vp, i32, vp, i32, i32, vp]),
    "svit_cast_f32_bf16": (i32, [vp, vp, i64, vp]),
    "svit_table_interp": (i32, [vp, i32, i32, vp, vp, vp, vp]),
    "svit_table_interp_batched": (i32, [vp, i32, i32, vp]),
    "svit_transpose_cast_batched": (i32, [vp, vp, vp, i32, i32, vp]),
    "svit_transpose_bf16_batched": (i32, [vp, vp, vp, i32, i32, vp]),
    "svit_scale_cast": (i32, [vp, vp, vp, i32, i64, i32, i32, i32, i32, vp]),
    "svit_pad_cast_rows": (i32, [vp, vp, i32, i32, i32, vp]),
    "svit_reduce_defer": (i32, [i32, vp]),
    "svit_reduce_flush": (i32, [vp]),
    "svit_reduce_reset": (i32, [vp]),
    "svit_layernorm_fwd": (i32, [vp, vp, vp, vp, vp, vp, vp, i64, i32, f32, vp]),
    "svit_layernorm_bwd": (i32, [vp, i32, vp, vp, vp, vp, vp, vp, vp, vp, i32, vp, vp, i64, i32, vp,
                                 i64, vp]),
    "svit_im2col_patch": (i32, [vp, vp, i32, i32, i32, i32, vp]),
    "svit_im2col_patch_u8": (i32, [vp, i64, vp, vp, vp, i32, i32, i32, i32, i32, vp]),
    "svit_im2col_patch_u8_mix": (i32, [vp, i64, vp, vp, vp, vp, i32, i32, i32, i32, i32, vp]),
    "svit_mixup_clips": (i32, [vp, vp, i32, i32, i32, i32, vp]),
    "svit_fill_special_tokens": (i32, [vp, vp, vp, vp, i32, i32, i32, i32, i32, i32, i32, vp]),
    "svit_special_token_grads": (i32, [vp, vp, vp, vp, i32, i32, i32, i32, i32, i32, i32, vp]),
    "svit_pool_ln_fwd": (i32, [C.POINTER(PoolArgs), vp]),
    "svit_pool_ln_bwd": (i32, [C.POINTER(PoolLnBwdArgs), vp]),
    "svit_pool_ln_fwd_qkv": (i32, [C.POINTER(PoolArgs), vp]),
    "svit_pool_ln_fwd_qkv_sel": (i32, [C.POINTER(PoolArgs), C.POINTER(vp), vp]),
    "svit_pool_weight_sel": (i32, [vp, vp, vp, i32, vp]),
    "svit_pool_ln_bwd_qkv": (i32, [C.POINTER(PoolLnBwdArgs), vp]),
    "svit_pool_conv_bwd_qkv": (i32, [C.POINTER(PoolDgradArgs), C.POINTER(PoolWgradArgs), vp]),
    "svit_pool_conv_bwd_workspace": (i64, [C.POINTER(PoolDgradArgs)]),
    "svit_relpos_q_fwd": (i32, [C.POINTER(RelqArgs), vp]),
    "svit_relpos_q_bwd": (i32, [C.POINTER(RelqBwdArgs), vp]),
    "svit_relpos_scatter": (i32, [C.POINTER(RelqScatterArgs), vp]),
    "svit_relpos_gather": (i32, [C.POINTER(RelqGatherArgs), vp]),
    "svit_attn_fwd": (i32, [C.POINTER(AttnFwdArgs), vp]),
    "svit_attn_bwd": (i32, [C.POINTER(AttnBwdArgs), vp]),
    "svit_attn_bwd_parts": (i32, [C.POINTER(AttnBwdArgs)]),
    "svit_maxpool_fwd": (i32, [vp, vp, vp, i32, i32, i32, i32, i32, i32, vp]),
    "svit_maxpool_bwd": (i32, [vp, vp, vp, i32, i32, i32, i32, i32, i32, vp]),
    "svit_maxpool_bwd_bf16": (i32, [vp, vp, vp, i32, i32, i32, i32, i32, i32, vp]),
    "svit_sumsq": (i32, [vp, i64, vp, vp, i64, vp]),
    "svit_adamw_step": (i32, [vp, vp, vp, vp, i64, vp, f32, f32, f32, f32, f32, f32, i32, f32, vp]),
    "svit_adamw_bias_table": (i32, [f32, f32, vp, i64, C.POINTER(i64)]),
    "svit_step_guard": (i32, [vp, i64, vp, vp, vp, i64, vp, i64, vp]),
    "svit_adamw_step_guarded": (i32, [vp, vp, vp, vp, i64, i64, vp, vp, f32, f32, f32, vp]),
    "svit_head_fwd": (i32, [C.POINTER(HeadArgs), vp]),
    "svit_head_bwd": (i32, [C.POINTER(HeadBwdArgs), vp]),
    "svit_haog_loss": (i32, [vp, vp, vp, vp, vp, vp, vp, vp, vp, i32, i32, vp]),
    "svit_haog_loss_bwd": (i32, [vp, vp, vp, vp, vp, vp, vp, i32, i32, vp]),
    "svit_ce_loss": (i32, [vp, vp, i32, i32, vp, vp, vp]),
    "svit_ce_loss_soft": (i32, [vp, vp, vp, vp, f32, f32, i32, i32, vp, vp, vp]),
    "svit_step_draws": (i32, [vp, vp, i32, i32, vp, i32, C.c_float, vp, vp]),
    "svit_ensemble_update": (i32, [vp, vp, vp, i32, i32, i32, i32, i32, i32, vp, vp, vp, vp, vp]),
    "svit_topk_correct": (i32, [vp, vp, i32, i32, vp, i32, vp, vp, vp]),
    "svit_debug_set": (i32, [i32, i32]),
    "svit_debug_set_tn": (i32, [i32, i32]),
    "svit_debug_set_tn_tile": (i32, [i32]),
    "svit_debug_set_pool": (i32, [i32, i32]),
    "svit_attn_debug_set": (i32, [i32, i32]),
    "svit_debug_reset": (i32, []),
    "svit_debug_pool_bwd_path": (i32, []),
}
EXPORTS = tuple(sorted(_SIGS))


class SvitHipError(RuntimeError):
    pass


def load():
    global _lib
    if _lib is None:
        if not os.path.exists(LIB_PATH):
            raise SvitHipError(
                "libsvit_hip.so not found at %s -- run `python -m svit_amd.build` "
                "(the SViT HIP path has no PyTorch/CPU fallback)" % LIB_PATH)
        if os.environ.get("SVIT_HIP_LIB"):
            import warnings
            warnings.warn("SVIT_HIP_LIB is set: loading the SViT HIP library from %s instead of the "
                          "in-tree build" % LIB_PATH)
        lib = C.CDLL(LIB_PATH)
        for name, (res, args) in _SIGS.items():
            fn = getattr(lib, name)
            fn.restype, fn.argtypes = res, args
        _lib = lib
    return _lib


_raw_stream = torch._C._cuda_getCurrentRawStream
_cur_device = torch._C._cuda_getDevice


def stream():
    return C.c_void_p(_raw_stream(_cur_device()))


def ptr(t):
    if t is None:
        return None
    return t.data_ptr()


def check(rc, what):
    if rc != 0:
        kind = {-2: "bad shape", -3: "bad alignment/stride", -4: "bad argument"}.get(
            rc, "hipError_t %d" % rc)
        raise SvitHipError("%s failed: %s" % (what, kind))


_trace = None


def start_trace():
    global _trace
    _trace = []


def stop_trace():
    global _trace
    t, _trace = _trace, None
    return t


def mark(label):
    if _trace is not None:
        e = torch.cuda.Event(enable_timing=True)
        e.record()
        _trace.append(("mark:" + label, e, e, None))


def call(name, *args, meta=None):
    if _trace is None:
        rc = getattr(load(), name)(*args, stream())
        check(rc, name)
        return
    e0 = torch.cuda.Event(enable_timing=True)
    e1 = torch.cuda.Event(enable_timing=True)
    e0.record()
    rc = getattr(load(), name)(*args, stream())
    e1.record()
    check(rc, name)
    _trace.append((name, e0, e1, meta))
```

svit_amd/ops.py:

```python
import ctypes as C

import torch

from . import hip
from .hip import ptr

BF16 = torch.bfloat16
F32 = torch.float32
HD = 96
_scratch = {}


def scratch(device, floats=8 * 1024 * 1024, tag="main"):
    key = (device.index, floats, tag)
    buf = _scratch.get(key)
    if buf is None:
        buf = torch.empty(floats, device=device, dtype=F32)
        _scratch[key] = buf
    return buf


def _chk_rows(*ts):
    for t in ts:
        if not t.is_cuda or t.dim() != 2 or t.stride(1) != 1:
            raise hip.SvitHipError("svit_amd GEMM operands must be 2-D device tensors with unit inner stride")


def _chk_dev(*ts):
    for t in ts:
        if t is not None and not t.is_cuda:
            raise hip.SvitHipError("svit_amd ops need device tensors (got %s)" % t.device)
        if t is not None and not t.is_contiguous():
            raise hip.SvitHipError("svit_amd ops need contiguous tensors")


def gemm_nt(a, w, bias=None, epilogue=hip.EPI_BF16, out=None, out2=None, aux=None,
            row_scale=None, rows_per_sample=0, accumulate=False, remap=None, save=True, relq=None):
    _chk_rows(a)
    _chk_dev(w, bias, out, out2, aux, row_scale)
    M, K = a.shape
    N = w.shape[0]
    assert w.shape[1] == K and a.dtype == BF16 and w.dtype == BF16
    if epilogue == hip.EPI_RELQ:
        cmap, qa, scale = relq
        _chk_dev(cmap, qa)
        extra = qa.shape[-1] - 96
        assert cmap.dtype == torch.int32 and cmap.is_contiguous() and cmap.shape == (qa.shape[-2], extra)
        assert qa.is_contiguous() and qa.numel() == M * qa.shape[-1] and bias is None
        g = hip.GemmArgs()
        g.A, g.lda, g.W, g.ldw = ptr(a), a.stride(0), ptr(w), w.stride(0)
        g.M, g.N, g.K, g.epilogue = M, N, K, epilogue
        g.relq_map, g.relq_out, g.relq_ld = ptr(cmap), ptr(qa), qa.shape[-1]
        g.relq_extra, g.relq_rows, g.relq_scale = extra, qa.shape[-2], scale
        hip.call("svit_gemm_nt", C.byref(g), meta=("mnk", M, N, K, epilogue, 2 * M * K + 2 * N * K + 2 * M * extra))
        return qa
    if out is None:
        dt = F32 if epilogue in (hip.EPI_RESID, hip.EPI_F32) else BF16
        out = torch.empty((M, N), device=a.device, dtype=dt)
    if epilogue == hip.EPI_GELU and out2 is None and save:
        out2 = torch.empty((M, N), device=a.device, dtype=BF16)
    g = hip.GemmArgs()
    g.A, g.lda, g.W, g.ldw = ptr(a), a.stride(0), ptr(w), w.stride(0)
    g.bias = ptr(bias)
    g.out, g.ldo = ptr(out), out.stride(-2)
    g.out2, g.ldo2 = ptr(out2), (out2.stride(-2) if out2 is not None else 0)
    g.aux, g.ldaux = ptr(aux), (aux.stride(-2) if aux is not None else 0)
    g.row_scale, g.rows_per_sample = ptr(row_scale), rows_per_sample
    g.M, g.N, g.K = M, N, K
    g.epilogue, g.accumulate = epilogue, int(accumulate)
    if remap is not None:
        g.remap_L, g.remap_N, g.remap_off = remap
    osz = out.element_size()
    nbytes = 2 * M * K + 2 * N * K + M * N * osz
    if out2 is not None:
        nbytes += 2 * M * N
    if aux is not None:
        nbytes += M * N * aux.element_size()
    if accumulate:
        nbytes += M * N * osz
    hip.call("svit_gemm_nt", C.byref(g), meta=("mnk", M, N, K, epilogue, nbytes))
    return (out, out2) if epilogue == hip.EPI_GELU else out


def gemm_tn(a, b, dw, splits=0, dbias=None):
    _chk_rows(a, b)
    _chk_dev(dw)
    M, N = a.shape
    K = dw.shape[-1]
    assert b.shape[0] == M and b.shape[1] >= K and dw.shape[-2] == N and dw.dtype == F32
    hip.call("svit_gemm_tn", ptr(a), a.stride(0), ptr(b), b.stride(0), ptr(dw), dw.stride(-2),
             M, N, K, splits, ptr(dbias), meta=("mnk", M, N, K))
    return dw


def gemm_tn_grouped(problems, ordered=False):
    n = len(problems)
    if n == 0:
        return
    arr = (hip.TnProblem * n)()
    flop = 0.0
    for i, (a, b, dw, dbias) in enumerate(problems):
        _chk_rows(a, b)
        _chk_dev(dw)
        M, N = a.shape
        K = dw.shape[-1]
        assert b.shape[0] == M and b.shape[1] >= K and dw.shape[-2] == N and dw.dtype == F32
        t = arr[i]
        t.A, t.B, t.dW, t.dbias = ptr(a), ptr(b), ptr(dw), ptr(dbias)
        t.lda, t.ldb, t.lddw, t.M, t.N, t.K = a.stride(0), b.stride(0), dw.stride(-2), M, N, K
        flop += 2.0 * M * N * K
    if ordered:
        hip.call("svit_gemm_tn_grouped_ex", arr, n, 1, meta=("flop", flop))
    else:
        hip.call("svit_gemm_tn_grouped", arr, n, meta=("flop", flop))


def _tn_problem_array(problems):
    n = len(problems)
    arr = (hip.TnProblem * n)()
    flop = 0.0
    for i, (a, b, dw, dbias) in enumerate(problems):
        _chk_rows(a, b, dw)
        _chk_dev(dbias)
        M, N = a.shape
        K = dw.shape[1]
        assert b.shape[0] == M and b.shape[1] >= K and dw.shape[0] == N and dw.dtype == F32
        t = arr[i]
        t.A, t.B, t.dW, t.dbias = ptr(a), ptr(b), ptr(dw), ptr(dbias)
        t.lda, t.ldb, t.lddw, t.M, t.N, t.K = a.stride(0), b.stride(0), dw.stride(0), M, N, K
        flop += 2.0 * M * N * K
    return arr, flop


_tn_slab_need = {}
_tn_slab_ws = {}


def gemm_tn_slab_workspace(arr, n, fresh=False):
    key = tuple((t.M, t.N, t.K, t.dbias is not None) for t in arr)
    need = None if fresh else _tn_slab_need.get(key)
    if need is None:
        need = hip.load().svit_gemm_tn_grouped_workspace(arr, n)
        if need < 0:
            hip.check(need, "svit_gemm_tn_grouped_workspace")
        _tn_slab_need[key] = need
    return need


def _tn_slab_buffer(dev, tag, need):
    key = (dev.index, tag)
    ws = _tn_slab_ws.get(key)
    if ws is None or ws.numel() < need:
        if ws is not None:
            torch.cuda.synchronize(dev)
        ws = _tn_slab_ws[key] = torch.empty(max(need, 1), device=dev, dtype=F32)
    return ws


def gemm_tn_grouped_slab(problems, ws=None, tag="tn_slab"):
    n = len(problems)
    if n == 0:
        return
    arr, flop = _tn_problem_array(problems)
    if ws is not None:
        _chk_dev(ws)
        assert ws.dtype == F32
        hip.call("svit_gemm_tn_grouped_slab", arr, n, ptr(ws), ws.numel(), meta=("flop", flop))
        return
    dev = problems[0][2].device
    ws = _tn_slab_buffer(dev, tag, gemm_tn_slab_workspace(arr, n))
    try:
        hip.call("svit_gemm_tn_grouped_slab", arr, n, ptr(ws), ws.numel(), meta=("flop", flop))
    except hip.SvitHipError:
        need = gemm_tn_slab_workspace(arr, n, fresh=True)
        if need <= ws.numel():
            raise
        ws = _tn_slab_buffer(dev, tag, need)
        hip.call("svit_gemm_tn_grouped_slab", arr, n, ptr(ws), ws.numel(), meta=("flop", flop))


def reduce_defer(on):
    hip.call("svit_reduce_defer", int(on))


def reduce_flush():
    hip.call("svit_reduce_flush")


def reduce_reset():
    hip.call("svit_reduce_reset")


def colsum(a, out):
    _chk_dev(a, out)
    hip.call("svit_colsum_bf16", ptr(a), a.stride(0), ptr(out), a.shape[0], a.shape[1])
    return out


def cast_bf16(src, dst=None):
    _chk_dev(src, dst)
    if dst is None:
        dst = torch.empty(src.shape, device=src.device, dtype=BF16)
    hip.call("svit_cast_f32_bf16", ptr(src), ptr(dst), src.numel())
    return dst


def transpose_cast_batched(src_flat, dst_flat, table, n_mats, max_tiles):
    hip.call("svit_transpose_cast_batched", ptr(src_flat), ptr(dst_flat), ptr(table), n_mats,
             max_tiles)


def transpose_bf16_batched(src16_flat, dst_flat, table, n_mats, max_tiles):
    _chk_dev(src16_flat, dst_flat, table)
    assert src16_flat.dtype == BF16 and dst_flat.dtype == BF16
    hip.call("svit_transpose_bf16_batched", ptr(src16_flat), ptr(dst_flat), ptr(table), n_mats,
             max_tiles)


def table_interp(mcat, tables, want_f32=True):
    _chk_dev(mcat, tables)
    assert mcat.dtype == F32 and tables.dtype == F32 and mcat.is_contiguous() and tables.is_contiguous()
    assert mcat.shape[1] == tables.shape[0] and tables.shape[1] == HD
    r32 = torch.empty((mcat.shape[0], HD), device=mcat.device, dtype=F32) if want_f32 else None
    r16 = torch.empty((mcat.shape[0], HD), device=mcat.device, dtype=BF16)
    hip.call("svit_table_interp", ptr(mcat), mcat.shape[0], mcat.shape[1], ptr(tables), ptr(r32), ptr(r16))
    return r32, r16


def table_interp_jobs(entries, device):
    import struct
    raw = b"".join(struct.pack("<QQQQii", ptr(m), ptr(t), ptr(o32) or 0, ptr(o16) or 0, m.shape[0], m.shape[1])
                   for m, t, o32, o16 in entries)
    return torch.frombuffer(bytearray(raw), dtype=torch.uint8).view(len(entries), 40).to(device)


def table_interp_batched(jobs, max_rows):
    hip.call("svit_table_interp_batched", ptr(jobs), jobs.shape[0], max_rows)


def pad_cast_rows(src, dst):
    _chk_dev(src, dst)
    hip.call("svit_pad_cast_rows", ptr(src), ptr(dst), src.shape[0], src.shape[1], dst.shape[1])
    return dst


def scale_cast(src, row_scale=None, rows_per_sample=0, dst=None, gather=None):
    _chk_dev(src, row_scale, dst)
    cols = src.shape[-1]
    if gather is None:
        rows, gl, gn, go = src.shape[:-1].numel(), 0, 0, 0
        shape = src.shape
    else:
        gl, go = gather
        gn = src.shape[-2]
        rows = src.shape[0] * gl
        shape = (rows, cols)
    if dst is None:
        dst = torch.empty(shape, device=src.device, dtype=BF16)
    hip.call("svit_scale_cast", ptr(src), ptr(dst), ptr(row_scale), rows_per_sample, rows, cols,
             gl, gn, go)
    return dst


def layernorm_fwd(x, gamma, beta, eps=1e-6, want_f32=False, want_bf16=True, save_stats=True):
    _chk_dev(x, gamma, beta)
    C_ = x.shape[-1]
    rows = x.numel() // C_
    y16 = torch.empty(x.shape, device=x.device, dtype=BF16) if want_bf16 else None
    y32 = torch.empty(x.shape, device=x.device, dtype=F32) if want_f32 else None
    mean = torch.empty(rows, device=x.device, dtype=F32) if save_stats else None
    rstd = torch.empty(rows, device=x.device, dtype=F32) if save_stats else None
    hip.call("svit_layernorm_fwd", ptr(x), ptr(gamma), ptr(beta), ptr(y16), ptr(y32), ptr(mean),
             ptr(rstd), rows, C_, eps)
    return y16, y32, mean, rstd


def layernorm_bwd(dy, x, gamma, mean, rstd, dgamma, dbeta, dres=None, dx=None, want_bf16=False,
                  row_scale=None, rows_per_sample=0, ws=None):
    _chk_dev(dy, x, gamma, mean, rstd, dgamma, dbeta, dres, dx, row_scale)
    C_ = x.shape[-1]
    rows = x.numel() // C_
    if dx is None:
        dx = torch.empty(x.shape, device=x.device, dtype=F32)
    dx16 = torch.empty(x.shape, device=x.device, dtype=BF16) if want_bf16 else None
    ws = scratch(x.device) if ws is None else ws
    assert dy.dtype in (F32, BF16)
    hip.call("svit_layernorm_bwd", ptr(dy), int(dy.dtype == BF16), ptr(x), ptr(gamma), ptr(mean),
             ptr(rstd), ptr(dres),
             ptr(dx), ptr(dx16), ptr(row_scale), rows_per_sample, ptr(dgamma), ptr(dbeta), rows, C_,
             ptr(ws), ws.numel())
    return (dx, dx16) if want_bf16 else dx


def im2col_patch(video):
    _chk_dev(video)
    B, Cin, T, H, W = video.shape
    assert Cin == 3 and video.dtype == F32
    To, Ho, Wo = (T - 1) // 2 + 1, (H - 1) // 4 + 1, (W - 1) // 4 + 1
    cols = torch.empty((B * To * Ho * Wo, 448), device=video.device, dtype=BF16)
    hip.call("svit_im2col_patch", ptr(video), ptr(cols), B, T, H, W)
    return cols, (To, Ho, Wo)


def im2col_patch_u8(clips):
    fr = clips.frames
    _chk_dev(fr)
    V, T, Hs, Ws, _ = fr.shape
    B, S = clips.crops.shape[0], clips.size
    To, Ho, Wo = (T - 1) // 2 + 1, (S - 1) // 4 + 1, (S - 1) // 4 + 1
    cols = torch.empty((B * To * Ho * Wo, 448), device=fr.device, dtype=BF16)
    mix = getattr(clips, "mix", None)
    if mix is not None:
        _chk_mix(mix, fr.device)
        hip.call("svit_im2col_patch_u8_mix", ptr(fr), fr.numel(), ptr(clips.lut_f32), ptr(clips.crops), ptr(mix),
                 ptr(cols), B, T, Hs, Ws, S)
        return cols, (To, Ho, Wo)
    hip.call("svit_im2col_patch_u8", ptr(fr), fr.numel(), ptr(clips.lut), ptr(clips.crops),
             ptr(cols), B, T, Hs, Ws, S)
    return cols, (To, Ho, Wo)


def _chk_mix(mix, device):
    _chk_dev(mix)
    if mix.dtype != torch.int32 or mix.numel() != 8 or mix.device != device:
        raise hip.SvitHipError("the mix record must be int32 [8] on %s (got %s %s on %s)"
                               % (device, mix.dtype, tuple(mix.shape), mix.device))


def mixup_clips(x, mix):
    _chk_dev(x)
    _chk_mix(mix, x.device)
    if x.dtype != F32 or x.dim() < 3:
        raise hip.SvitHipError("mixup_clips needs an fp32 [B, ..., H, W] tensor, got %s %s" % (x.dtype, tuple(x.shape)))
    B, H, W = x.shape[0], x.shape[-2], x.shape[-1]
    hip.call("svit_mixup_clips", ptr(x), ptr(mix), B, x[0].numel() // (H * W), H, W)
    return x


def fill_special_tokens(x, cls, objq, pos_t, L, Tx, O, add_pos):
    B, N, C_ = x.shape
    hip.call("svit_fill_special_tokens", ptr(x), ptr(cls), ptr(objq), ptr(pos_t), B, N, L, Tx, O,
             C_, int(add_pos))


def special_token_grads(dx, g_cls, g_obj, g_pos, L, Tx, O, add_pos):
    B, N, C_ = dx.shape
    assert dx.is_contiguous() and dx.dtype == F32
    hip.call("svit_special_token_grads", ptr(dx), ptr(g_cls), ptr(g_obj), ptr(g_pos), B, N, L, Tx, O, C_, int(add_pos))


def pooled(n, s):
    return (n - 1) // s + 1


NOGRAD_SCRATCH = True


def _pool_fwd_args(a, qkv, which, conv_w, gamma, beta, B, heads, thw, n_obj, stride_hw, ld_out, mode,
                   eps, save=True, out_scale=1.0):
    _chk_dev(qkv, conv_w, gamma, beta)
    T, H, W = thw
    Nout = 1 + T * pooled(H, stride_hw) * pooled(W, stride_hw) + n_obj
    dev = qkv.device
    out = torch.empty((B, heads, Nout, ld_out), device=dev, dtype=BF16)
    keep = save or (NOGRAD_SCRATCH and T > 1)
    pre = torch.empty((B, heads, Nout, HD), device=dev, dtype=BF16) if keep else None
    mean = torch.empty(B * heads * Nout, device=dev, dtype=F32) if keep else None
    rstd = torch.empty(B * heads * Nout, device=dev, dtype=F32) if keep else None
    a.qkv, a.which, a.conv_w, a.gamma, a.beta = ptr(qkv), which, ptr(conv_w), ptr(gamma), ptr(beta)
    a.out, a.ld_out, a.pre, a.mean, a.rstd = ptr(out), ld_out, ptr(pre), ptr(mean), ptr(rstd)
    a.B, a.heads, a.T, a.H, a.W, a.n_obj = B, heads, T, H, W, n_obj
    a.stride_hw, a.mode, a.eps, a.out_scale = stride_hw, mode, eps, out_scale
    return out, pre, mean, rstd


def pool_ln_fwd(qkv, which, conv_w, gamma, beta, B, heads, thw, n_obj, stride_hw, ld_out=HD,
                mode=0, eps=1e-6, out_scale=1.0):
    a = hip.PoolArgs()
    res = _pool_fwd_args(a, qkv, which, conv_w, gamma, beta, B, heads, thw, n_obj, stride_hw,
                         ld_out, mode, eps, out_scale=out_scale)
    hip.call("svit_pool_ln_fwd", C.byref(a))
    return res


def pool_weight_sel(src_flat, offsets, dst):
    _chk_dev(src_flat, offsets, dst)
    hip.call("svit_pool_weight_sel", ptr(src_flat), ptr(offsets), ptr(dst), offsets.numel())
    return dst


def _sel_ptrs(sels):
    arr = (C.c_void_p * 3)()
    for i in range(3):
        arr[i] = ptr(sels[i])
    return arr


def pool_ln_fwd_qkv(qkv, conv_ws, gammas, betas, B, heads, thw, n_obj, strides, ld_outs, modes,
                    eps=1e-6, save=True, sels=None, out_scales=(1.0, 1.0, 1.0), relq=None):
    arr = (hip.PoolArgs * 3)()
    res = [_pool_fwd_args(arr[i], qkv, i, conv_ws[i], gammas[i], betas[i], B, heads, thw, n_obj,
                          strides[i], ld_outs[i], modes[i], eps, save, out_scale=out_scales[i])
           for i in range(3)]
    if relq is not None:
        rcat, cmap, rscale = relq
        _chk_dev(rcat, cmap)
        assert rcat.dtype == BF16 and rcat.is_contiguous() and rcat.shape[1] == HD
        assert cmap.dtype == torch.int32 and cmap.is_contiguous()
        assert tuple(cmap.shape) == (res[0][0].shape[2], ld_outs[0] - HD)
        arr[0].relq_R, arr[0].relq_map, arr[0].relq_lpad, arr[0].relq_scale = ptr(rcat), ptr(cmap), rcat.shape[0], rscale
    if sels is None:
        hip.call("svit_pool_ln_fwd_qkv", arr)
    else:
        hip.call("svit_pool_ln_fwd_qkv_sel", arr, _sel_ptrs(sels))
    if not save:
        res = [(r[0], None, None, None) for r in res]
    return res


def _pool_ln_bwd_args(a, pre, mean, rstd, gamma, dgamma, dbeta, B, heads, Nout, d_main=None,
                      ld_main=HD, d_res=None, d_extra=None, ws=None):
    dpre = torch.empty((B, heads, Nout, HD), device=pre.device, dtype=BF16)
    a.d_main = ptr(d_main)
    a.main_is_f32 = int(d_main is not None and d_main.dtype == F32)
    a.ld_main = ld_main
    a.main_parts, a.main_part_stride = 1, 0
    if d_main is not None and d_main.dim() == 5:
        assert d_main.dtype == F32
        a.main_parts, a.main_part_stride = d_main.shape[0], d_main.stride(0)
    a.d_res, a.d_extra = ptr(d_res), ptr(d_extra)
    a.extra_is_bf16 = int(d_extra is not None and d_extra.dtype == BF16)
    a.pre, a.mean, a.rstd, a.gamma = ptr(pre), ptr(mean), ptr(rstd), ptr(gamma)
    a.dpre, a.dgamma, a.dbeta = ptr(dpre), ptr(dgamma), ptr(dbeta)
    a.B, a.heads, a.Nout = B, heads, Nout
    ws = scratch(pre.device) if ws is None else ws
    a.workspace, a.workspace_floats = ptr(ws), ws.numel()
    return dpre


def pool_ln_bwd(pre, mean, rstd, gamma, dgamma, dbeta, B, heads, Nout, d_main=None, ld_main=HD,
                d_res=None, d_extra=None):
    a = hip.PoolLnBwdArgs()
    dpre = _pool_ln_bwd_args(a, pre, mean, rstd, gamma, dgamma, dbeta, B, heads, Nout, d_main,
                             ld_main, d_res, d_extra)
    hip.call("svit_pool_ln_bwd", C.byref(a))
    return dpre


def pool_ln_bwd_qkv(entries, ws=None):
    arr = (hip.PoolLnBwdArgs * 3)()
    res = [_pool_ln_bwd_args(arr[i], *entries[i][0], ws=ws, **entries[i][1]) for i in range(3)]
    hip.call("svit_pool_ln_bwd_qkv", arr)
    return res


def _pool_dgrad_args(a, dpre, conv_w, dqkv, which, B, heads, thw, n_obj, stride_hw):
    a.dpre, a.conv_w, a.dqkv, a.which = ptr(dpre), ptr(conv_w), ptr(dqkv), which
    a.B, a.heads, (a.T, a.H, a.W), a.n_obj, a.stride_hw = B, heads, thw, n_obj, stride_hw




def _pool_wgrad_args(a, dpre, qkv, which, dw, B, heads, thw, n_obj, stride_hw, ws=None):
    a.dpre, a.qkv, a.which, a.dw = ptr(dpre), ptr(qkv), which, ptr(dw)
    a.B, a.heads, (a.T, a.H, a.W), a.n_obj, a.stride_hw = B, heads, thw, n_obj, stride_hw
    ws = scratch(dpre.device) if ws is None else ws
    a.workspace, a.workspace_floats = ptr(ws), ws.numel()




def pool_conv_bwd_workspace(B, heads, thw, n_obj, strides):
    da = (hip.PoolDgradArgs * 3)()
    for i in range(3):
        da[i].B, da[i].heads, (da[i].T, da[i].H, da[i].W), da[i].n_obj, da[i].stride_hw, da[i].which = B, heads, thw, n_obj, strides[i], i
    return int(hip.load().svit_pool_conv_bwd_workspace(da))


def pool_conv_bwd_qkv(dpres, conv_ws, dqkv, qkv, dws, B, heads, thw, n_obj, strides, ws=None):
    if ws is None:
        need = pool_conv_bwd_workspace(B, heads, thw, n_obj, strides)
        ws = scratch(dpres[0].device, max(8 * 1024 * 1024, need), tag="poolbwd")
    da = (hip.PoolDgradArgs * 3)()
    wa = (hip.PoolWgradArgs * 3)()
    for i in range(3):
        _pool_dgrad_args(da[i], dpres[i], conv_ws[i], dqkv, i, B, heads, thw, n_obj, strides[i])
        _pool_wgrad_args(wa[i], dpres[i], qkv, i, dws[i], B, heads, thw, n_obj, strides[i], ws)
    hip.call("svit_pool_conv_bwd_qkv", da, wa)


def relpos_q_fwd(qa, tabs, idx, B, heads, q_thw, k_thw, n_obj, inv_scale):
    a = hip.RelqArgs()
    a.qa, a.ld = ptr(qa), qa.shape[-1]
    a.rel_h, a.rel_w, a.rel_t = (ptr(t) for t in tabs)
    a.idx_h, a.idx_w, a.idx_t = (ptr(t) for t in idx)
    a.B, a.heads = B, heads
    a.qt, a.qh, a.qw = q_thw
    a.kt, a.kh, a.kw = k_thw
    a.n_obj, a.inv_scale = n_obj, inv_scale
    hip.call("svit_relpos_q_fwd", C.byref(a))


def relpos_q_bwd(qa, dqa, tabs, idx, dtabs, B, heads, q_thw, k_thw, n_obj, inv_scale):
    Nq = qa.shape[2]
    dq_extra = torch.empty((B, heads, Nq, HD), device=qa.device, dtype=F32)
    a = hip.RelqBwdArgs()
    a.qa, a.dqa, a.ld = ptr(qa), ptr(dqa), qa.shape[-1]
    a.rel_h, a.rel_w, a.rel_t = (ptr(t) for t in tabs)
    a.idx_h, a.idx_w, a.idx_t = (ptr(t) for t in idx)
    a.dq_extra = ptr(dq_extra)
    a.drel_h, a.drel_w, a.drel_t = (ptr(t) for t in dtabs)
    a.rows_h, a.rows_w, a.rows_t = (t.shape[0] for t in tabs)
    a.B, a.heads = B, heads
    a.qt, a.qh, a.qw = q_thw
    a.kt, a.kh, a.kw = k_thw
    a.n_obj, a.inv_scale = n_obj, inv_scale
    ws = scratch(qa.device)
    a.workspace, a.workspace_floats = ptr(ws), ws.numel()
    hip.call("svit_relpos_q_bwd", C.byref(a))
    return dq_extra


def relpos_gather(P, qa, idx, rows_off, B, heads, q_thw, k_thw, n_obj, inv_scale):
    a = hip.RelqGatherArgs()
    a.P, a.ldp, a.qa, a.ld = ptr(P), P.shape[-1], ptr(qa), qa.shape[-1]
    a.idx_h, a.idx_w, a.idx_t = (ptr(t) for t in idx)
    a.row_h, a.row_w, a.row_t = rows_off
    a.B, a.heads = B, heads
    a.qt, a.qh, a.qw = q_thw
    a.kt, a.kh, a.kw = k_thw
    a.n_obj, a.inv_scale = n_obj, inv_scale
    hip.call("svit_relpos_gather", C.byref(a))


def relpos_scatter(dqa, idx, offs, ldd, B, heads, q_thw, k_thw, n_obj, inv_scale):
    Nq = dqa.shape[2]
    D = torch.empty((B * heads * Nq, ldd), device=dqa.device, dtype=BF16)
    a = hip.RelqScatterArgs()
    a.dqa, a.ld, a.D, a.ldd = ptr(dqa), dqa.shape[-1], ptr(D), ldd
    a.idx_h, a.idx_w, a.idx_t = (ptr(t) for t in idx)
    a.off_h, a.off_w, a.off_t = offs
    a.B, a.heads = B, heads
    a.qt, a.qh, a.qw = q_thw
    a.kt, a.kh, a.kw = k_thw
    a.n_obj, a.inv_scale = n_obj, inv_scale
    hip.call("svit_relpos_scatter", C.byref(a))
    return D


def attn_fwd(qa, ka, v, scale, bias_cols=0):
    _chk_dev(qa, ka, v)
    B, heads, Nq, DA = qa.shape
    Nk = ka.shape[2]
    ctx = torch.empty((B, Nq, heads * HD), device=qa.device, dtype=BF16)
    lse2 = torch.empty((B, heads, Nq), device=qa.device, dtype=F32)
    a = hip.AttnFwdArgs()
    a.qa, a.ka, a.v, a.ctx, a.lse2 = ptr(qa), ptr(ka), ptr(v), ptr(ctx), ptr(lse2)
    a.B, a.heads, a.Nq, a.Nk, a.DA, a.scale, a.bias_cols = B, heads, Nq, Nk, DA, scale, bias_cols
    hip.call("svit_attn_fwd", C.byref(a), meta=("attn", B, heads, Nq, Nk, DA))
    return ctx, lse2


def attn_bwd(qa, ka, v, ctx, dctx, lse2, scale, q_splits=0, bias_cols=0, reld=None):
    _chk_dev(qa, ka, v, ctx, dctx, lse2)
    B, heads, Nq, DA = qa.shape
    Nk = ka.shape[2]
    dev = qa.device
    a = hip.AttnBwdArgs()
    a.B, a.heads, a.Nq, a.Nk, a.DA, a.q_splits, a.scale = B, heads, Nq, Nk, DA, q_splits, scale
    a.bias_cols = bias_cols
    parts = hip.load().svit_attn_bwd_parts(C.byref(a))
    if parts < 1:
        raise hip.SvitHipError("svit_attn_bwd_parts failed: %d" % parts)
    dqa = torch.empty((B, heads, Nq, DA), device=dev, dtype=BF16)
    dkv = torch.empty((2, parts, B, heads, Nk, HD), device=dev, dtype=F32)
    delta = torch.empty((B, heads, Nq, 2), device=dev, dtype=F32)
    a.qa, a.ka, a.v, a.ctx, a.dctx, a.lse2 = (ptr(t) for t in (qa, ka, v, ctx, dctx, lse2))
    a.delta, a.dqa, a.dk, a.dv = ptr(delta), ptr(dqa), ptr(dkv[0]), ptr(dkv[1])
    a.q_splits = parts
    D = X = None
    if reld is not None:
        cmap, ldd, rscale = reld[:3]
        rt = reld[3] if len(reld) > 3 else None
        _chk_dev(cmap, rt)
        assert cmap.dtype == torch.int32 and cmap.is_contiguous() and cmap.shape == (Nq, DA - HD)
        D = torch.empty((B * heads * Nq, ldd), device=dev, dtype=BF16)
        a.relD, a.relD_ld, a.relD_map, a.relD_scale = ptr(D), ldd, ptr(cmap), rscale
        mode = reld[4] if len(reld) > 4 else "separate"
        if rt is not None and ldd <= 128 and ldd % 16 == 0:
            assert rt.dtype == BF16 and rt.is_contiguous() and tuple(rt.shape) == (HD, ldd)
            a.relR = ptr(rt)
            if mode == "fold":
                X = "folded"
            else:
                X = torch.empty((B * heads * Nq, HD), device=dev, dtype=F32)
                a.relX = ptr(X)
    folded = 2.0 * B * heads * Nq * HD * reld[1] if (reld is not None and X is not None) else 0.0
    hip.call("svit_attn_bwd", C.byref(a), meta=("attn", B, heads, Nq, Nk, DA, folded))
    if reld is not None:
        return dqa, dkv[0], dkv[1], D, X
    return dqa, dkv[0], dkv[1]


def maxpool_fwd(x, thw, n_obj):
    B, N, C_ = x.shape
    T, H, W = thw
    Nout = 1 + T * pooled(H, 2) * pooled(W, 2) + n_obj
    y = torch.empty((B, Nout, C_), device=x.device, dtype=F32)
    idx = torch.empty((B, Nout, C_), device=x.device, dtype=torch.uint8)
    hip.call("svit_maxpool_fwd", ptr(x), ptr(y), ptr(idx), B, T, H, W, n_obj, C_)
    return y, idx


def maxpool_bwd(dy, idx, thw, n_obj, bf16=False):
    B, Nout, C_ = dy.shape
    T, H, W = thw
    dx = torch.empty((B, 1 + T * H * W + n_obj, C_), device=dy.device, dtype=BF16 if bf16 else F32)
    hip.call("svit_maxpool_bwd_bf16" if bf16 else "svit_maxpool_bwd", ptr(dy), ptr(idx), ptr(dx),
             B, T, H, W, n_obj, C_)
    return dx


def sumsq(g, out):
    ws = scratch(g.device)
    hip.call("svit_sumsq", ptr(g), g.numel(), ptr(out), ptr(ws), ws.numel())


def adamw_step(p, g, m, v, sumsq_t, max_norm, lr, beta1, beta2, eps, wd, step, grad_scale=1.0):
    hip.call("svit_adamw_step", ptr(p), ptr(g), ptr(m), ptr(v), p.numel(), ptr(sumsq_t), max_norm,
             lr, beta1, beta2, eps, wd, step, grad_scale)


def adamw_bias_table(beta1, beta2):
    import numpy as np
    cap = 1 << 20
    buf = np.empty((cap, 2), dtype=np.float32)
    n = C.c_int64(0)
    rc = hip.load().svit_adamw_bias_table(beta1, beta2, buf.ctypes.data, cap, C.byref(n))
    hip.check(rc, "svit_adamw_bias_table (betas %r, %r)" % (beta1, beta2))
    return buf[:n.value].copy()


def _chk_step_records(host_rec, dev_rec, device):
    _chk_dev(host_rec, dev_rec)
    if (host_rec.dtype != F32 or host_rec.numel() != 8 or dev_rec.dtype != torch.int32 or dev_rec.numel() != 12
            or host_rec.device != device or dev_rec.device != device):
        raise hip.SvitHipError("the step record is fp32 [8] + int32 [12] on %s" % (device,))


def step_guard(g, host_rec, dev_rec, table, workspace):
    _chk_dev(g, table, workspace)
    _chk_step_records(host_rec, dev_rec, g.device)
    hip.call("svit_step_guard", ptr(g), g.numel(), ptr(host_rec), ptr(dev_rec), ptr(table), table.shape[0],
             ptr(workspace), workspace.numel())


def adamw_step_guarded(p, g, m, v, n_decay, host_rec, dev_rec, beta1, beta2, eps):
    _chk_dev(p, g, m, v)
    _chk_step_records(host_rec, dev_rec, p.device)
    n = p.numel()
    if g.numel() != n or m.numel() != n or v.numel() != n:
        raise hip.SvitHipError("adamw_step_guarded: p, g, m, v differ in size")
    hip.call("svit_adamw_step_guarded", ptr(p), ptr(g), ptr(m), ptr(v), n, n_decay, ptr(host_rec), ptr(dev_rec),
             beta1, beta2, eps)


def _head_args(tokens, T, O, keep, head_params, outs):
    a = hip.HeadArgs()
    B, N, C_ = tokens.shape
    a.tokens, a.B, a.N, a.C, a.T, a.O = ptr(tokens), B, N, C_, T, O
    a.keep = ptr(keep)
    (wp, bp), (wb, bb), (we, be), (wc, bc) = head_params
    a.w_proj, a.b_proj, a.n_cls = ptr(wp), ptr(bp), wp.shape[0]
    a.w_box, a.b_box, a.w_bce, a.b_bce, a.w_con, a.b_con = ptr(wb), ptr(bb), ptr(we), ptr(be), ptr(wc), ptr(bc)
    a.logits, a.boxes, a.contact, a.xobj = (ptr(t) for t in outs)
    return a


def head_fwd(tokens, T, O, keep, head_params):
    assert tokens.is_contiguous() and tokens.dtype == F32
    _chk_dev(tokens, keep, *[t for wb in head_params for t in wb])
    B, N, C_ = tokens.shape
    dev = tokens.device
    outs = (torch.empty((B, head_params[0][0].shape[0]), device=dev), torch.empty((B, T, O, 5), device=dev),
            torch.empty((B, T, 2, 5), device=dev), torch.empty((B, T, O, C_), device=dev))
    a = _head_args(tokens, T, O, keep, head_params, outs)
    hip.call("svit_head_fwd", C.byref(a))
    return outs


def head_bwd(tokens, T, O, keep, head_params, boxes, grads_out, param_grads, ordered=False):
    assert tokens.is_contiguous() and tokens.dtype == F32
    go = [None if t is None else t.contiguous() for t in grads_out]
    _chk_dev(tokens, keep, boxes, *[t for t in go if t is not None])
    g = hip.HeadBwdArgs()
    g.f = _head_args(tokens, T, O, keep, head_params, (boxes, boxes, boxes, None))
    g.dlogits, g.dboxes, g.dcontact, g.dxobj = (ptr(t) for t in go)
    dtok = torch.empty_like(tokens)
    g.dtokens = ptr(dtok)
    (gwp, gbp), (gwb, gbb), (gwe, gbe), (gwc, gbc) = param_grads
    g.gw_proj, g.gb_proj, g.gw_box, g.gb_box = ptr(gwp), ptr(gbp), ptr(gwb), ptr(gbb)
    g.gw_bce, g.gb_bce, g.gw_con, g.gb_con = ptr(gwe), ptr(gbe), ptr(gwc), ptr(gbc)
    g.ordered = int(ordered)
    hip.call("svit_head_bwd", C.byref(g))
    return dtok


def haog_loss_fwd(pred, tar, contact, contact_tar):
    R, Rc = pred.numel() // 5, contact.numel() // 5
    assert pred.dtype == F32 and tar.dtype == F32 and contact.dtype == F32
    assert contact_tar.dtype == torch.int64 and tar.numel() == R * 4 and contact_tar.numel() == Rc
    dev = pred.device
    losses = torch.empty(8, dtype=F32, device=dev)
    g_l1, g_giou = torch.empty((R, 4), dtype=F32, device=dev), torch.empty((R, 4), dtype=F32, device=dev)
    g_bce, g_contact = torch.empty(R, dtype=F32, device=dev), torch.empty((Rc, 5), dtype=F32, device=dev)
    hip.call("svit_haog_loss", ptr(pred), ptr(tar), ptr(contact), ptr(contact_tar), ptr(losses),
             ptr(g_l1), ptr(g_bce), ptr(g_giou), ptr(g_contact), R, Rc)
    return losses, (g_l1, g_bce, g_giou, g_contact)


def haog_loss_bwd(upstream, unit, pred_shape, contact_shape):
    g_l1, g_bce, g_giou, g_contact = unit
    R, Rc = g_bce.numel(), g_contact.numel() // 5
    dpred = torch.empty(pred_shape, dtype=F32, device=g_bce.device)
    dcontact = torch.empty(contact_shape, dtype=F32, device=g_bce.device)
    hip.call("svit_haog_loss_bwd", ptr(upstream), ptr(g_l1), ptr(g_bce), ptr(g_giou),
             ptr(g_contact), ptr(dpred), ptr(dcontact), R, Rc)
    return dpred, dcontact


def ce_loss(logits, labels):
    _chk_dev(logits, labels)
    assert logits.dtype == F32 and logits.dim() == 2 and labels.dtype == torch.int64 and labels.numel() == logits.shape[0]
    logits, labels = logits.contiguous(), labels.contiguous()
    loss = torch.empty((), device=logits.device, dtype=F32)
    dlogits = torch.empty_like(logits)
    hip.call("svit_ce_loss", ptr(logits), ptr(labels), logits.shape[0], logits.shape[1], ptr(loss), ptr(dlogits))
    return loss, dlogits


def ce_loss_soft(logits, target=None, labels=None, mix=None, on=1.0, off=0.0):
    _chk_dev(logits, target, labels)
    assert logits.dtype == F32 and logits.dim() == 2
    B, C_ = logits.shape
    if (target is None) == (labels is None):
        raise hip.SvitHipError("ce_loss_soft takes a dense target or labels, not both / neither")
    if target is not None:
        assert target.dtype == F32 and target.shape == logits.shape and mix is None
    else:
        assert labels.dtype == torch.int64 and labels.numel() == B
        if mix is not None:
            _chk_mix(mix, logits.device)
    loss = torch.empty((), device=logits.device, dtype=F32)
    dlogits = torch.empty_like(logits)
    hip.call("svit_ce_loss_soft", ptr(logits), ptr(target), ptr(labels), ptr(mix), float(on), float(off), B, C_,
             ptr(loss), ptr(dlogits))
    return loss, dlogits


def step_draws(state, keep, per_block, n_drop=0, p_drop=0.0):
    _chk_dev(state, keep)
    assert state.dtype == torch.int64 and state.numel() == 3 and keep.dtype == F32
    nb = keep.numel()
    scales = torch.empty((nb, per_block), device=state.device, dtype=F32)
    drop = torch.empty((n_drop,), device=state.device, dtype=F32) if n_drop else None
    hip.call("svit_step_draws", ptr(state), ptr(keep), nb, per_block, ptr(scales), n_drop, float(p_drop), ptr(drop))
    return scales, drop
```

Measured before the change: 683.8 clips/s.

## Skip GEMM tiles and LayerNorm rows for samples dropped by DropPath

Passes the per-sample DropPath scale into the NT GEMM and the LayerNorm forward/backward kernels. GEMM workgroups whose row tile covers only dropped samples write the value the epilogue would produce (zeros, or the residual copy) and return without loading or multiplying. LayerNorm rows of dropped samples skip their loads and write zeros, or pass the residual gradient straight through in backward. This removes compute on residual branches whose output is multiplied by zero, at the cost of extra per-tile checks and a dependence on how many samples are dropped each step.

```diff
diff --git a/include/svit_hip.h b/include/svit_hip.h
--- a/include/svit_hip.h
+++ b/include/svit_hip.h
@@ -33,6 +33,7 @@
   void* relq_out; int32_t relq_ld;
   int32_t relq_extra, relq_rows;
   float relq_scale;
+  const float* skip_scale; int32_t skip_rows;
 } svit_gemm_args;
 int svit_gemm_nt(const svit_gemm_args* args, void* stream);
 int svit_gemm_tn(const void* A, int lda, const void* B, int ldb, float* dW, int lddw,
@@ -76,12 +77,20 @@
 int svit_layernorm_fwd(const float* x, const float* gamma, const float* beta, void* y_bf16,
                        float* y_f32, float* mean, float* rstd, int64_t rows, int C, float eps,
                        void* stream);
+int svit_layernorm_fwd_ex(const float* x, const float* gamma, const float* beta, void* y_bf16,
+                          float* y_f32, float* mean, float* rstd, int64_t rows, int C, float eps,
+                          const float* skip_scale, int skip_rows, void* stream);
 int svit_layernorm_bwd(const void* dy , int dy_is_bf16,
                        const float* x, const float* gamma, const float* mean,
                        const float* rstd, const float* dres, float* dx, void* dx_bf16,
                        const float* row_scale, int rows_per_sample, float* dgamma,
                        float* dbeta, int64_t rows, int C, float* workspace,
                        int64_t workspace_floats, void* stream);
+int svit_layernorm_bwd_ex(const void* dy, int dy_is_bf16, const float* x, const float* gamma,
+                          const float* mean, const float* rstd, const float* dres, float* dx,
+                          void* dx_bf16, const float* row_scale, int rows_per_sample, float* dgamma,
+                          float* dbeta, int64_t rows, int C, float* workspace, int64_t workspace_floats,
+                          const float* skip_scale, int skip_rows, void* stream);
 
 int svit_im2col_patch(const float* video, void* cols, int B, int T, int H, int W, void* stream);
 int svit_im2col_patch_u8(const uint8_t* frames, int64_t frames_bytes, const void* lut,
diff --git a/svit_amd/csrc/gemm_epilogue.h b/svit_amd/csrc/gemm_epilogue.h
--- a/svit_amd/csrc/gemm_epilogue.h
+++ b/svit_amd/csrc/gemm_epilogue.h
@@ -277,3 +277,51 @@
     if (ih + 1 < 2 * RB) nt_epi_sync<WAVE_PRIVATE>();
   }
 }
+
+__device__ __forceinline__ bool nt_tile_dead(const svit_gemm_args& p, int m0, int BM) {
+  if (!p.skip_scale) return false;
+  const int s_first = m0 / p.skip_rows, s_last = (min(m0 + BM, p.M) - 1) / p.skip_rows;
+  bool dead = true;
+  for (int s = s_first; s <= s_last; ++s) dead = dead && (p.skip_scale[s] == 0.0f);
+  return dead;
+}
+
+template <int EPI>
+__device__ __forceinline__ void nt_dead_store(const svit_gemm_args& p, int m0, int n0, int BM, int BN, int tid, int nt) {
+  const int rows = min(BM, p.M - m0), cols = min(BN, p.N - n0);
+  if constexpr (EPI == SVIT_EPI_RELQ) {
+    if (n0 != 0) return;
+    bf16_t* qa = (bf16_t*)p.relq_out;
+    const int e = p.relq_extra;
+    for (int i = tid; i < rows * e; i += nt) qa[(size_t)(m0 + i / e) * p.relq_ld + 96 + i % e] = 0;
+  } else if constexpr (EPI == SVIT_EPI_RESID) {
+    const int c4 = cols / 4;
+    for (int i = tid; i < rows * c4; i += nt) {
+      const size_t r = (size_t)(m0 + i / c4);
+      const int c = n0 + 4 * (i % c4);
+      *(float4*)((float*)p.out + r * p.ldo + c) = *(const float4*)((const float*)p.aux + r * p.ldaux + c);
+    }
+  } else if constexpr (EPI == SVIT_EPI_F32) {
+    if (p.accumulate) return;
+    const int c4 = cols / 4;
+    for (int i = tid; i < rows * c4; i += nt) {
+      const int row = m0 + i / c4;
+      const size_t r = p.remap_L > 0 ? (size_t)(row / p.remap_L) * p.remap_N + p.remap_off + (row % p.remap_L) : (size_t)row;
+      *(float4*)((float*)p.out + r * p.ldo + n0 + 4 * (i % c4)) = make_float4(0.f, 0.f, 0.f, 0.f);
+    }
+  } else {
+    auto zero_bf16 = [&](bf16_t* out, int ld) {
+      if (ld % 8 == 0) {
+        const int c8 = cols / 8;
+        for (int i = tid; i < rows * c8; i += nt)
+          *(uint4*)(out + (size_t)(m0 + i / c8) * ld + n0 + 8 * (i % c8)) = make_uint4(0u, 0u, 0u, 0u);
+      } else {
+        const int c4 = cols / 4;
+        for (int i = tid; i < rows * c4; i += nt)
+          *(uint2*)(out + (size_t)(m0 + i / c4) * ld + n0 + 4 * (i % c4)) = make_uint2(0u, 0u);
+      }
+    };
+    zero_bf16((bf16_t*)p.out, p.ldo);
+    if (EPI == SVIT_EPI_GELU && p.out2) zero_bf16((bf16_t*)p.out2, p.ldo2);
+  }
+}
diff --git a/svit_amd/csrc/gemm_nt.hip b/svit_amd/csrc/gemm_nt.hip
--- a/svit_amd/csrc/gemm_nt.hip
+++ b/svit_amd/csrc/gemm_nt.hip
@@ -32,6 +32,11 @@
   const int xq = nwg >> 3, xr = nwg & 7, xcd = lin & 7;
   const int wgid = (xcd < xr ? xcd * (xq + 1) : xr * (xq + 1) + (xcd - xr) * xq) + (lin >> 3);
   const int m0 = (wgid / gridDim.x) * BM, n0 = (wgid % gridDim.x) * BN;
+
+  if (nt_tile_dead(p, m0, BM)) {
+    nt_dead_store<EPI>(p, m0, n0, BM, BN, tid, NT);
+    return;
+  }
 
   const bf16_t* src[PER];
 #pragma unroll
@@ -201,6 +206,11 @@
   const int m0 = (wgid / gridDim.x) * BM, n0 = (wgid % gridDim.x) * BN;
   const int nk = p.K / 64;
 
+  if (nt_tile_dead(p, m0, BM)) {
+    nt_dead_store<EPI>(p, m0, n0, BM, BN, (int)threadIdx.x, (NC + NL) * 64);
+    return;
+  }
+
   if (wave >= NC) {
     nt_ring_loader<NL, BM, BN, STAGES>(p, smem, wave - NC, lane, m0, n0, nk);
     return;
@@ -334,6 +344,7 @@
   if (a.out2 && (a.ldo2 % 4 != 0 || ((uintptr_t)a.out2 & 15))) return SVIT_ERR_ALIGN;
   if ((a.epilogue == SVIT_EPI_RESID || a.epilogue == SVIT_EPI_DGELU) && !a.aux) return SVIT_ERR_ARG;
   if (a.epilogue == SVIT_EPI_RESID && a.row_scale && a.rows_per_sample <= 0) return SVIT_ERR_ARG;
+  if (a.skip_scale && a.skip_rows <= 0) return SVIT_ERR_ARG;
   hipStream_t st = (hipStream_t)stream;
   const int force_raw = svit_knob(SVIT_K_NT_CFG), force_stages = svit_knob(SVIT_K_NT_STAGES);
   const bool no_ring = force_raw == 8 || svit_knob(SVIT_K_NT_BK) != 0;
diff --git a/svit_amd/csrc/norm.hip b/svit_amd/csrc/norm.hip
--- a/svit_amd/csrc/norm.hip
+++ b/svit_amd/csrc/norm.hip
@@ -21,7 +21,8 @@
                                                      float* __restrict__ y32,
                                                      float* __restrict__ mean_out,
                                                      float* __restrict__ rstd_out, int64_t rows,
-                                                     int C, float eps) {
+                                                     int C, float eps,
+                                                     const float* __restrict__ skip, int skip_rows) {
   constexpr int LW = HALF ? 32 : 64;
   constexpr int RPW = HALF ? 2 : 1;
   const int lane = threadIdx.x & 63, wave = threadIdx.x >> 6;
@@ -39,16 +40,20 @@
   for (int64_t row0 = ((int64_t)blockIdx.x * 4 + wave) * RPW + sub; row0 < rows; row0 += 2 * stride) {
     float4 v[2][NCH];
     int64_t rk[2];
-    bool has[2];
+    bool has[2], dead[2];
 #pragma unroll
     for (int k = 0; k < 2; ++k) {
       has[k] = row0 + k * stride < rows;
       rk[k] = has[k] ? row0 + k * stride : row0;
+      dead[k] = skip && skip[(uint32_t)rk[k] / (uint32_t)skip_rows] == 0.0f;
+    }
+#pragma unroll
+    for (int k = 0; k < 2; ++k) {
 #pragma unroll
       for (int i = 0; i < NCH; ++i) {
         const int c = lr + i * LW;
         v[k][i] = make_float4(0.f, 0.f, 0.f, 0.f);
-        if (c < nch) v[k][i] = ((const float4*)(x + rk[k] * C))[c];
+        if (c < nch && !dead[k]) v[k][i] = ((const float4*)(x + rk[k] * C))[c];
       }
     }
 #pragma unroll
@@ -69,8 +74,8 @@
       const float rstd = rsqrtf(row_sum<HALF>(sq) * inv_c + eps);
       if (!has[k]) continue;
       if (lr == 0) {
-        if (mean_out) mean_out[rk[k]] = mean;
-        if (rstd_out) rstd_out[rk[k]] = rstd;
+        if (mean_out) mean_out[rk[k]] = dead[k] ? 0.f : mean;
+        if (rstd_out) rstd_out[rk[k]] = dead[k] ? 0.f : rstd;
       }
 #pragma unroll
       for (int i = 0; i < NCH; ++i) {
@@ -81,6 +86,7 @@
           o.y = (v[k][i].y - mean) * rstd * g[i].y + bt[i].y;
           o.z = (v[k][i].z - mean) * rstd * g[i].z + bt[i].z;
           o.w = (v[k][i].w - mean) * rstd * g[i].w + bt[i].w;
+          if (dead[k]) o = make_float4(0.f, 0.f, 0.f, 0.f);
           if (y16) {
             uint2 pk;
             pk.x = pack_bf16x2(o.x, o.y);
@@ -106,7 +112,8 @@
                                                      const float* __restrict__ row_scale,
                                                      int rows_per_sample,
                                                      float* __restrict__ partial,
-                                                     int64_t rows, int C) {
+                                                     int64_t rows, int C,
+                                                     const float* __restrict__ skip, int skip_rows) {
   constexpr int LW = HALF ? 32 : 64;
   constexpr int RPW = HALF ? 2 : 1;
   __shared__ float red[4][2][NCH * 256];
@@ -127,19 +134,25 @@
     float4 xv[2][NCH], dv[2][NCH], rv[2][NCH];
     float mean[2], rstd[2], sc16[2];
     int64_t rowk[2];
-    bool has[2];
+    bool has[2], dead[2];
 #pragma unroll
     for (int k = 0; k < 2; ++k) {
       has[k] = row0 + k * stride < rows;
       rowk[k] = has[k] ? row0 + k * stride : row0;
-      mean[k] = mean_in[rowk[k]];
-      rstd[k] = rstd_in[rowk[k]];
+      dead[k] = skip && skip[(uint32_t)rowk[k] / (uint32_t)skip_rows] == 0.0f;
+    }
+#pragma unroll
+    for (int k = 0; k < 2; ++k) {
+      mean[k] = dead[k] ? 0.f : mean_in[rowk[k]];
+      rstd[k] = dead[k] ? 0.f : rstd_in[rowk[k]];
       sc16[k] = (dx16 && row_scale) ? row_scale[rowk[k] / rows_per_sample] : 1.f;
 #pragma unroll
       for (int i = 0; i < NCH; ++i) {
         const int c = lr + i * LW;
         xv[k][i] = dv[k][i] = rv[k][i] = make_float4(0.f, 0.f, 0.f, 0.f);
-        if (c < nch) {
+        if (c < nch && dead[k]) {
+          if (dres) rv[k][i] = ((const float4*)(dres + rowk[k] * C))[c];
+        } else if (c < nch) {
           xv[k][i] = ((const float4*)(x + rowk[k] * C))[c];
           if (DYB) {
             const uint2 h = ((const uint2*)((const bf16_t*)dy_ + rowk[k] * C))[c];
@@ -183,6 +196,7 @@
           o.y = rstd[k] * (g[i].y - s1 - xh[i].y * s2) + rv[k][i].y;
           o.z = rstd[k] * (g[i].z - s1 - xh[i].z * s2) + rv[k][i].z;
           o.w = rstd[k] * (g[i].w - s1 - xh[i].w * s2) + rv[k][i].w;
+          if (dead[k]) o = rv[k][i];
           ((float4*)(dx + rowk[k] * C))[c] = o;
           if (dx16) {
             uint2 h;
@@ -220,10 +234,12 @@
 }
 }
 
-extern "C" int svit_layernorm_fwd(const float* x, const float* gamma, const float* beta,
-                                  void* y_bf16, float* y_f32, float* mean, float* rstd,
-                                  int64_t rows, int C, float eps, void* stream) {
+extern "C" int svit_layernorm_fwd_ex(const float* x, const float* gamma, const float* beta,
+                                     void* y_bf16, float* y_f32, float* mean, float* rstd,
+                                     int64_t rows, int C, float eps, const float* skip_scale,
+                                     int skip_rows, void* stream) {
   if (!x || !gamma || !beta || (!y_bf16 && !y_f32)) return SVIT_ERR_ARG;
+  if (skip_scale && (skip_rows <= 0 || rows > 0x7fffffff)) return SVIT_ERR_ARG;
   if (rows <= 0 || C <= 0 || C % 4 != 0 || C > 768) return SVIT_ERR_SHAPE;
   constexpr int rpb_f = 8;
   int64_t blocks = (rows + rpb_f - 1) / rpb_f;
@@ -232,7 +248,7 @@
 #define SVIT_LN_FWD(NCH, HALF)                                                                \
   hipLaunchKernelGGL((ln_fwd_kernel<NCH, HALF>), dim3((unsigned)blocks), dim3(256), 0,           \
                      (hipStream_t)stream, x, gamma, beta, (bf16_t*)y_bf16, y_f32, mean, rstd,    \
-                     rows, C, eps)
+                     rows, C, eps, skip_scale, skip_rows)
   if (C <= 128) SVIT_LN_FWD(1, true);
   else if (C <= 256) SVIT_LN_FWD(1, false);
   else if (C <= 512) SVIT_LN_FWD(2, false);
@@ -242,14 +258,21 @@
   return SVIT_OK;
 }
 
-extern "C" int svit_layernorm_bwd(const void* dy, int dy_is_bf16, const float* x, const float* gamma,
-                                  const float* mean, const float* rstd, const float* dres,
-                                  float* dx, void* dx_bf16, const float* row_scale,
-                                  int rows_per_sample, float* dgamma, float* dbeta, int64_t rows,
-                                  int C, float* workspace, int64_t workspace_floats,
-                                  void* stream) {
+extern "C" int svit_layernorm_fwd(const float* x, const float* gamma, const float* beta,
+                                  void* y_bf16, float* y_f32, float* mean, float* rstd,
+                                  int64_t rows, int C, float eps, void* stream) {
+  return svit_layernorm_fwd_ex(x, gamma, beta, y_bf16, y_f32, mean, rstd, rows, C, eps, nullptr, 0, stream);
+}
+
+extern "C" int svit_layernorm_bwd_ex(const void* dy, int dy_is_bf16, const float* x, const float* gamma,
+                                     const float* mean, const float* rstd, const float* dres,
+                                     float* dx, void* dx_bf16, const float* row_scale,
+                                     int rows_per_sample, float* dgamma, float* dbeta, int64_t rows,
+                                     int C, float* workspace, int64_t workspace_floats,
+                                     const float* skip_scale, int skip_rows, void* stream) {
   if (!dy || !x || !gamma || !mean || !rstd || !dx || !dgamma || !dbeta || !workspace)
     return SVIT_ERR_ARG;
+  if (skip_scale && (skip_rows <= 0 || rows > 0x7fffffff)) return SVIT_ERR_ARG;
   if (dx_bf16 && row_scale && rows_per_sample <= 0) return SVIT_ERR_ARG;
   if (rows <= 0 || C <= 0 || C % 4 != 0 || C > 768) return SVIT_ERR_SHAPE;
   constexpr int rpb = 16;
@@ -263,11 +286,13 @@
     if (dy_is_bf16)                                                                               \
       hipLaunchKernelGGL((ln_bwd_kernel<NCH, HALF, true>), dim3((unsigned)blocks), dim3(256), 0,  \
                          (hipStream_t)stream, dy, x, gamma, mean, rstd, dres, dx,                 \
-                         (bf16_t*)dx_bf16, row_scale, rows_per_sample, workspace, rows, C);       \
+                         (bf16_t*)dx_bf16, row_scale, rows_per_sample, workspace, rows, C,  \
+                         skip_scale, skip_rows);      \
     else                                                                                          \
       hipLaunchKernelGGL((ln_bwd_kernel<NCH, HALF, false>), dim3((unsigned)blocks), dim3(256), 0, \
                          (hipStream_t)stream, dy, x, gamma, mean, rstd, dres, dx,                 \
-                         (bf16_t*)dx_bf16, row_scale, rows_per_sample, workspace, rows, C);       \
+                         (bf16_t*)dx_bf16, row_scale, rows_per_sample, workspace, rows, C,  \
+                         skip_scale, skip_rows);      \
   } while (0)
   if (C <= 128) SVIT_LN_BWD(1, true);
   else if (C <= 256) SVIT_LN_BWD(1, false);
@@ -280,3 +305,13 @@
   SVIT_LAUNCH_CHECK();
   return SVIT_OK;
 }
+
+extern "C" int svit_layernorm_bwd(const void* dy, int dy_is_bf16, const float* x, const float* gamma,
+                                  const float* mean, const float* rstd, const float* dres,
+                                  float* dx, void* dx_bf16, const float* row_scale,
+                                  int rows_per_sample, float* dgamma, float* dbeta, int64_t rows,
+                                  int C, float* workspace, int64_t workspace_floats,
+                                  void* stream) {
+  return svit_layernorm_bwd_ex(dy, dy_is_bf16, x, gamma, mean, rstd, dres, dx, dx_bf16, row_scale, rows_per_sample,
+                               dgamma, dbeta, rows, C, workspace, workspace_floats, nullptr, 0, stream);
+}
diff --git a/svit_amd/engine.py b/svit_amd/engine.py
--- a/svit_amd/engine.py
+++ b/svit_amd/engine.py
@@ -174,6 +174,7 @@
         self.attn_q_splits = 0
         self.deterministic = False
         self.reproducible = False
+        self.skip_dropped = True
         self._capture_fork = None
         self._capture_join = None
 
@@ -255,6 +256,9 @@
             t = self.flat.p(n)
             out.append(t if m is None else (m @ t).contiguous())
         return out
+
+    def _live(self, scale, rows):
+        return (scale, rows) if (self.skip_dropped and scale is not None) else None
 
     def forward(self, video, drop_scales=None, save=True):
         plan, f = self.plan, self.flat
@@ -306,10 +310,12 @@
         DA = HD + 32 if J <= 32 else HD + 64
         if J > 64:
             raise hip.SvitHipError("key grid %s too large for the in-MFMA rel-pos bias" % (k_thw,))
+        dpa, dpm = ds if ds is not None else (None, None)
         xn, _, mean1, rstd1 = ops.layernorm_fwd(x, f.p(pre + "norm1.weight"), f.p(pre + "norm1.bias"),
-                                                save_stats=save)
+                                                save_stats=save, skip=None if blk.has_proj else self._live(dpa, N))
         xn2d = xn.view(B * N, C)
-        qkv = ops.gemm_nt(xn2d, f.w(pre + "attn.qkv.weight"), f.p(pre + "attn.qkv.bias"), hip.EPI_BF16)
+        qkv = ops.gemm_nt(xn2d, f.w(pre + "attn.qkv.weight"), f.p(pre + "attn.qkv.bias"), hip.EPI_BF16,
+                          skip=self._live(dpa, N))
         idx, mats, mcat, need = self._rel(blk, q_thw, k_thw)
         if mcat is None:
             tabs = self._tables(pre, mats)
@@ -340,16 +346,17 @@
             skip = x
         if blk.pools_q:
             skip, pool_idx = ops.maxpool_fwd(skip, thw, n_obj)
-        dpa, dpm = ds if ds is not None else (None, None)
         x1 = ops.gemm_nt(ctx.view(B * Nq, Co), f.w(pre + "attn.proj.weight"), f.p(pre + "attn.proj.bias"),
-                         hip.EPI_RESID, aux=skip.view(B * Nq, Co), row_scale=dpa, rows_per_sample=Nq)
+                         hip.EPI_RESID, aux=skip.view(B * Nq, Co), row_scale=dpa, rows_per_sample=Nq,
+                         skip=self._live(dpa, Nq))
         x1 = x1.view(B, Nq, Co)
+        live_m = self._live(dpm, Nq)
         xn2, _, mean2, rstd2 = ops.layernorm_fwd(x1, f.p(pre + "norm2.weight"), f.p(pre + "norm2.bias"),
-                                                 save_stats=save)
+                                                 save_stats=save, skip=live_m)
         act, dact = ops.gemm_nt(xn2.view(B * Nq, Co), f.w(pre + "mlp.fc1.weight"),
-                                f.p(pre + "mlp.fc1.bias"), hip.EPI_GELU, save=save)
+                                f.p(pre + "mlp.fc1.bias"), hip.EPI_GELU, save=save, skip=live_m)
         x2 = ops.gemm_nt(act, f.w(pre + "mlp.fc2.weight"), f.p(pre + "mlp.fc2.bias"), hip.EPI_RESID,
-                         aux=x1.view(B * Nq, Co), row_scale=dpm, rows_per_sample=Nq).view(B, Nq, Co)
+                         aux=x1.view(B * Nq, Co), row_scale=dpm, rows_per_sample=Nq, skip=live_m).view(B, Nq, Co)
         sv = None
         if save:
             sv = dict(x=x, thw=thw, q_thw=q_thw, k_thw=k_thw, mean1=mean1, rstd1=rstd1, xn=xn2d,
@@ -463,12 +470,12 @@
             ops.gemm_tn(a, b, dw, splits=0, dbias=dbias)
 
     def _linear_bwd(self, dy16, x16, wname, bname, need_dx, out=None, accumulate=False,
-                    epilogue=hip.EPI_F32, aux=None):
+                    epilogue=hip.EPI_F32, aux=None, skip=None):
         f = self.flat
         self._tn.append((dy16, x16, f.g(wname), f.g(bname)))
         if not need_dx:
             return None
-        return ops.gemm_nt(dy16, f.wt(wname), None, epilogue, out=out, aux=aux, accumulate=accumulate)
+        return ops.gemm_nt(dy16, f.wt(wname), None, epilogue, out=out, aux=aux, accumulate=accumulate, skip=skip)
 
     def _block_bwd(self, blk, sv, dx2, dy, n_obj, below, red_begin=True, red_end=True, red_slot=0):
         f = self.flat
@@ -483,17 +490,18 @@
         if red_begin:
             ops.reduce_defer(True)
         dy = dy.view(Mq, Co)
+        live_m, live_a = self._live(sv["dpm"], Nq), self._live(sv["dpa"], Nq)
         dh = self._linear_bwd(dy, sv["act"], pre + "mlp.fc2.weight", pre + "mlp.fc2.bias", True,
-                              epilogue=hip.EPI_DGELU, aux=sv["dact"])
+                              epilogue=hip.EPI_DGELU, aux=sv["dact"], skip=live_m)
         dxn2 = self._linear_bwd(dh, sv["xn2"].view(Mq, Co), pre + "mlp.fc1.weight",
-                                pre + "mlp.fc1.bias", True, epilogue=hip.EPI_BF16)
+                                pre + "mlp.fc1.bias", True, epilogue=hip.EPI_BF16, skip=live_m)
         dx1, dy = ops.layernorm_bwd(dxn2, sv["x1"], f.p(pre + "norm2.weight"), sv["mean2"],
                                     sv["rstd2"], f.g(pre + "norm2.weight"), f.g(pre + "norm2.bias"),
                                     dres=dx2, want_bf16=True, row_scale=sv["dpa"], rows_per_sample=Nq,
-                                    ws=self._rws("ln2"))
+                                    ws=self._rws("ln2"), skip=live_m)
         dy = dy.view(Mq, Co)
         dctx = self._linear_bwd(dy, sv["ctx"].view(Mq, Co), pre + "attn.proj.weight",
-                                pre + "attn.proj.bias", True, epilogue=hip.EPI_BF16)
+                                pre + "attn.proj.bias", True, epilogue=hip.EPI_BF16, skip=live_a)
         (qa, preq, mq, rq), (ka, prek, mk, rk), (v, prev, mv, rv) = sv["pools"]
         tabs, mats = sv["tabs"], sv["mats"]
         names = (pre + "attn.rel_pos_h", pre + "attn.rel_pos_w", pre + "attn.rel_pos_t")
@@ -527,7 +535,7 @@
                 self._gemm_tn(D[:, o:o + rows], qa2[:, :HD], d)
                 f.g(n).add_(m.t() @ d)
         if dq_extra is None:
-            dq_extra = ops.gemm_nt(D, rcat_t, None, hip.EPI_BF16)
+            dq_extra = ops.gemm_nt(D, rcat_t, None, hip.EPI_BF16, skip=self._live(sv["dpa"], h * Nq))
         elif isinstance(dq_extra, str):
             dq_extra = None
         Nk = ka.shape[2]
@@ -548,7 +556,7 @@
                               [f.g(pre + "attn.pool_%s.weight" % r).view(HD, 27) for r in "qkv"],
                               B, h, thw, n_obj, strides, ws=self._wgrad_ws(B, h, thw, n_obj, strides))
         dxn = self._linear_bwd(dqkv, sv["xn"], pre + "attn.qkv.weight", pre + "attn.qkv.bias", True,
-                               epilogue=hip.EPI_F32 if blk.has_proj else hip.EPI_BF16)
+                               epilogue=hip.EPI_F32 if blk.has_proj else hip.EPI_BF16, skip=self._live(sv["dpa"], N))
         dskip = dx1
         if blk.pools_q:
             dskip = ops.maxpool_bwd(dskip, sv["pool_idx"], thw, n_obj, bf16=blk.has_proj)
@@ -561,7 +569,8 @@
                                 f.g(pre + "norm1.weight"), f.g(pre + "norm1.bias"), dres=dskip,
                                 want_bf16=below is not None,
                                 row_scale=below["dpm"] if below is not None else None,
-                                rows_per_sample=N, ws=self._rws("ln1"))
+                                rows_per_sample=N, ws=self._rws("ln1"),
+                                skip=None if blk.has_proj else self._live(sv["dpa"], N))
         if red_end:
             ops.reduce_defer(False)
         self._flush_tn(force=False)
diff --git a/svit_amd/hip.py b/svit_amd/hip.py
--- a/svit_amd/hip.py
+++ b/svit_amd/hip.py
@@ -23,7 +23,8 @@
                 ("row_scale", vp), ("rows_per_sample", i32), ("M", i32), ("N", i32), ("K", i32),
                 ("epilogue", i32), ("accumulate", i32), ("remap_L", i32), ("remap_N", i32),
                 ("remap_off", i32), ("relq_map", vp), ("relq_out", vp), ("relq_ld", i32),
-                ("relq_extra", i32), ("relq_rows", i32), ("relq_scale", f32)]
+                ("relq_extra", i32), ("relq_rows", i32), ("relq_scale", f32),
+                ("skip_scale", vp), ("skip_rows", i32)]
 
 
 class PoolArgs(C.Structure):
@@ -144,6 +145,9 @@
     "svit_layernorm_fwd": (i32, [vp, vp, vp, vp, vp, vp, vp, i64, i32, f32, vp]),
     "svit_layernorm_bwd": (i32, [vp, i32, vp, vp, vp, vp, vp, vp, vp, vp, i32, vp, vp, i64, i32, vp,
                                  i64, vp]),
+    "svit_layernorm_fwd_ex": (i32, [vp, vp, vp, vp, vp, vp, vp, i64, i32, f32, vp, i32, vp]),
+    "svit_layernorm_bwd_ex": (i32, [vp, i32, vp, vp, vp, vp, vp, vp, vp, vp, i32, vp, vp, i64, i32, vp,
+                                    i64, vp, i32, vp]),
     "svit_im2col_patch": (i32, [vp, vp, i32, i32, i32, i32, vp]),
     "svit_im2col_patch_u8": (i32, [vp, i64, vp, vp, vp, i32, i32, i32, i32, i32, vp]),
     "svit_im2col_patch_u8_mix": (i32, [vp, i64, vp, vp, vp, vp, i32, i32, i32, i32, i32, vp]),
diff --git a/svit_amd/ops.py b/svit_amd/ops.py
--- a/svit_amd/ops.py
+++ b/svit_amd/ops.py
@@ -34,10 +34,22 @@
             raise hip.SvitHipError("svit_amd ops need contiguous tensors")
 
 
+def _chk_skip(skip, rows):
+    if skip is None or skip[0] is None:
+        return None, 0
+    scale, per = skip
+    _chk_dev(scale)
+    if scale.dtype != F32 or per <= 0 or scale.numel() * per < rows:
+        raise hip.SvitHipError("DropPath liveness: %d fp32 factors x %d rows do not cover %d rows"
+                               % (scale.numel(), per, rows))
+    return scale, int(per)
+
+
 def gemm_nt(a, w, bias=None, epilogue=hip.EPI_BF16, out=None, out2=None, aux=None,
-            row_scale=None, rows_per_sample=0, accumulate=False, remap=None, save=True, relq=None):
+            row_scale=None, rows_per_sample=0, accumulate=False, remap=None, save=True, relq=None, skip=None):
     _chk_rows(a)
     _chk_dev(w, bias, out, out2, aux, row_scale)
+    skip_scale, skip_rows = _chk_skip(skip, a.shape[0])
     M, K = a.shape
     N = w.shape[0]
     assert w.shape[1] == K and a.dtype == BF16 and w.dtype == BF16
@@ -52,6 +64,7 @@
         g.M, g.N, g.K, g.epilogue = M, N, K, epilogue
         g.relq_map, g.relq_out, g.relq_ld = ptr(cmap), ptr(qa), qa.shape[-1]
         g.relq_extra, g.relq_rows, g.relq_scale = extra, qa.shape[-2], scale
+        g.skip_scale, g.skip_rows = ptr(skip_scale), skip_rows
         hip.call("svit_gemm_nt", C.byref(g), meta=("mnk", M, N, K, epilogue, 2 * M * K + 2 * N * K + 2 * M * extra))
         return qa
     if out is None:
@@ -68,6 +81,7 @@
     g.row_scale, g.rows_per_sample = ptr(row_scale), rows_per_sample
     g.M, g.N, g.K = M, N, K
     g.epilogue, g.accumulate = epilogue, int(accumulate)
+    g.skip_scale, g.skip_rows = ptr(skip_scale), skip_rows
     if remap is not None:
         g.remap_L, g.remap_N, g.remap_off = remap
     osz = out.element_size()
@@ -262,21 +276,26 @@
     return dst
 
 
-def layernorm_fwd(x, gamma, beta, eps=1e-6, want_f32=False, want_bf16=True, save_stats=True):
+def layernorm_fwd(x, gamma, beta, eps=1e-6, want_f32=False, want_bf16=True, save_stats=True, skip=None):
     _chk_dev(x, gamma, beta)
     C_ = x.shape[-1]
     rows = x.numel() // C_
+    skip_scale, skip_rows = _chk_skip(skip, rows)
     y16 = torch.empty(x.shape, device=x.device, dtype=BF16) if want_bf16 else None
     y32 = torch.empty(x.shape, device=x.device, dtype=F32) if want_f32 else None
     mean = torch.empty(rows, device=x.device, dtype=F32) if save_stats else None
     rstd = torch.empty(rows, device=x.device, dtype=F32) if save_stats else None
-    hip.call("svit_layernorm_fwd", ptr(x), ptr(gamma), ptr(beta), ptr(y16), ptr(y32), ptr(mean),
-             ptr(rstd), rows, C_, eps)
+    if skip_scale is None:
+        hip.call("svit_layernorm_fwd", ptr(x), ptr(gamma), ptr(beta), ptr(y16), ptr(y32), ptr(mean),
+                 ptr(rstd), rows, C_, eps)
+    else:
+        hip.call("svit_layernorm_fwd_ex", ptr(x), ptr(gamma), ptr(beta), ptr(y16), ptr(y32), ptr(mean),
+                 ptr(rstd), rows, C_, eps, ptr(skip_scale), skip_rows)
     return y16, y32, mean, rstd
 
 
 def layernorm_bwd(dy, x, gamma, mean, rstd, dgamma, dbeta, dres=None, dx=None, want_bf16=False,
-                  row_scale=None, rows_per_sample=0, ws=None):
+                  row_scale=None, rows_per_sample=0, ws=None, skip=None):
     _chk_dev(dy, x, gamma, mean, rstd, dgamma, dbeta, dres, dx, row_scale)
     C_ = x.shape[-1]
     rows = x.numel() // C_
@@ -285,10 +304,14 @@
     dx16 = torch.empty(x.shape, device=x.device, dtype=BF16) if want_bf16 else None
     ws = scratch(x.device) if ws is None else ws
     assert dy.dtype in (F32, BF16)
-    hip.call("svit_layernorm_bwd", ptr(dy), int(dy.dtype == BF16), ptr(x), ptr(gamma), ptr(mean),
-             ptr(rstd), ptr(dres),
-             ptr(dx), ptr(dx16), ptr(row_scale), rows_per_sample, ptr(dgamma), ptr(dbeta), rows, C_,
-             ptr(ws), ws.numel())
+    skip_scale, skip_rows = _chk_skip(skip, rows)
+    args = (ptr(dy), int(dy.dtype == BF16), ptr(x), ptr(gamma), ptr(mean), ptr(rstd), ptr(dres),
+            ptr(dx), ptr(dx16), ptr(row_scale), rows_per_sample, ptr(dgamma), ptr(dbeta), rows, C_,
+            ptr(ws), ws.numel())
+    if skip_scale is None:
+        hip.call("svit_layernorm_bwd", *args)
+    else:
+        hip.call("svit_layernorm_bwd_ex", *args, ptr(skip_scale), skip_rows)
     return (dx, dx16) if want_bf16 else dx
 
 
```

Result: no change. 681.1 clips/s (-0.4%).
